# uc-vision/taichi_gaussian_rasterizer

Hardware: AMD Instinct MI355X
Metric: Mpixels/s fwd+bwd @ 2048x2048, 1M Gaussians (higher is better)
Workload: dtype f32

## Files before the change

taichi_gaussian_rasterizer_amd/csrc/frame.cpp:

```cpp

#include <string.h>

#include "gs_common.h"

namespace {

int64_t a256(int64_t bytes) { return gs_align_up(bytes > 0 ? bytes : 1, 256); }

struct Dims {
  int64_t n, P, T;
  int C, F, col0, RS, tiles_x, tiles_y, local_h, D;
  bool want_vis;
};

int frame_dims(const GsFrame* f, Dims* d) {
  GS_REQUIRE(f != nullptr, GS_ERR_INVALID_ARGUMENT, "frame: descriptor is NULL");
  if (int rc = gs_check_cfg(&f->cfg)) return rc;
  GS_REQUIRE(f->n >= 0 && f->n < (int64_t(1) << 31), GS_ERR_INVALID_ARGUMENT, "frame: %lld gaussians", (long long)f->n);
  GS_REQUIRE(f->width > 0 && f->height > 0, GS_ERR_INVALID_ARGUMENT, "frame: image size %dx%d", f->width, f->height);
  GS_REQUIRE(f->sh_degree >= -1 && f->sh_degree <= 3, GS_ERR_UNSUPPORTED, "frame: SH degree %d", f->sh_degree);
  GS_REQUIRE(f->channels >= 1 && f->channels <= (f->sh_degree >= 0 ? GS_MAX_SH_CHANNELS : GS_MAX_FEATURES - 2),
             GS_ERR_UNSUPPORTED, "frame: %d feature channels", f->channels);
  const int ts = f->cfg.tile_size;
  GsShard sh;
  if (int rc = gs_make_shard(f->has_shard ? &f->shard : nullptr, int(gs_div_up(f->height, ts)), &sh)) return rc;
  d->n = f->n;
  d->C = f->channels;
  d->F = f->channels + (f->render_depth ? 2 : 0);
  d->col0 = d->F - d->C;
  d->RS = gs_grad_row_floats(d->F);
  d->D = f->sh_degree >= 0 ? (f->sh_degree + 1) * (f->sh_degree + 1) : 1;
  d->tiles_x = int(gs_div_up(f->width, ts));
  d->tiles_y = sh.local_rows;
  int64_t rows = 0;
  if (!f->has_shard) rows = f->height;
  else
    for (int l = 0; l < sh.local_rows; ++l) {
      const int gy = gs_shard_global_row(sh, l);
      const int64_t y0 = int64_t(gy) * ts, y1 = y0 + ts < f->height ? y0 + ts : f->height;
      rows += y1 - y0;
    }
  d->local_h = int(rows);
  d->T = int64_t(d->tiles_x) * d->tiles_y;
  d->P = rows * f->width;
  d->want_vis = f->cfg.compute_visibility || f->cfg.compute_point_heuristic;
  return GS_OK;
}

template <typename T>
T* at(void* base, int64_t off) { return reinterpret_cast<T*>(static_cast<char*>(base) + off); }

struct StageTimer {
  void* const* events;
  int rc = GS_OK;
  void mark(int stage, int end, void* stream) {
    if (!events || !events[2 * stage + end]) return;
    if (hipEventRecord(static_cast<hipEvent_t>(events[2 * stage + end]), static_cast<hipStream_t>(stream)) != hipSuccess) {
      gs_set_error("frame: hipEventRecord of a stage timer failed");
      rc = GS_ERR_LAUNCH;
    }
  }
};

}

int gs_project_fwd_ex(int64_t n, const float* position, const float* log_scaling, const float* rotation,
                      const float* alpha_logit, const float* T_camera_world, const float* projection, int32_t width,
                      int32_t height, double near_plane, double far_plane, const GsRasterConfig* cfg, float* points,
                      float* depth, float* ndc_depth, int64_t* indexes, int32_t* slot_of, int32_t* num_visible,
                      float* depth_features, int32_t depth_features_stride, float* camera_pos, void* scratch,
                      int64_t scratch_bytes, float* zero_rows, int32_t zero_row_floats, const GsMapBinPlan* bin,
                      void* stream);

extern "C" int gs_frame_layout(const GsFrame* f, GsFrameLayout* out) {
  Dims d;
  if (int rc = frame_dims(f, &d)) return rc;
  GS_REQUIRE(out != nullptr, GS_ERR_INVALID_ARGUMENT, "gs_frame_layout: layout is NULL");
  GS_REQUIRE(f->k_capacity >= 1, GS_ERR_INVALID_ARGUMENT, "gs_frame_layout: k_capacity must be >= 1");
  memset(out, 0, sizeof(*out));
  int64_t p = 0;
  auto take = [&](int64_t bytes) { const int64_t o = p; p += a256(bytes); return o; };
  const int64_t n = d.n > 0 ? d.n : 1;
  out->counts = take(8 * 4);
  out->camera_pos = take(3 * 4);
  out->points = take(n * 7 * 4);
  out->depth = take(n * 4);
  out->features = take(n * d.F * 4);
  out->indexes = take(n * 8);
  out->slot_of = take(n * 4);
  out->tile_ranges = take(d.T * 8);
  out->tile_order = take(d.T * 4);
  out->overlap_to_point = take(f->k_capacity * 4);
  out->image = take(d.P * d.F * 4);
  out->alpha = take(d.P * 4);
  out->visibility = d.want_vis ? take(n * 4) : -1;
  out->out_image = f->render_depth ? take(d.P * d.C * 4) : -1;
  out->img_depth = f->render_depth ? take(d.P * 4) : -1;
  out->img_var = f->render_depth ? take(d.P * 4) : -1;
  out->median = f->render_median_depth ? take(d.P * 4) : -1;
  out->grad_rows = f->prepare_backward ? take(n * d.RS * 4) : -1;
  const bool lists = f->has_shard && f->exchange_world > 0;
  out->touched = lists ? take(n * 4) : -1;
  out->owner_counts = lists ? take(64 * 8) : -1;
  out->workspace_bytes = p;
  p = 0;
  out->s_ndc_depth = take(n * 4);
  out->s_pairs = take(f->k_capacity * 8);
  out->s_median_cover = f->render_median_depth ? take(d.P * 4) : -1;
  const int64_t pb = gs_project_scratch_bytes(d.n), mb = gs_map_scratch_bytes(d.n, d.T > 0 ? d.T : 1);
  out->s_stage = take(a256(mb) + pb);
  out->stage_bytes = a256(mb) + pb;
  out->fwd_scratch_bytes = p;
  p = 0;
  out->b_grad_image = f->render_depth ? take(d.P * d.F * 4) : -1;
  out->b_camera = take(gs_project_bwd_scratch_bytes(d.n));
  out->b_grad_rows = f->prepare_backward ? -1 : take(n * d.RS * 4);
  out->bwd_scratch_bytes = p;
  out->num_features = d.F;
  out->grad_row_floats = d.RS;
  out->tiles_x = d.tiles_x;
  out->tiles_y = d.tiles_y;
  out->local_height = d.local_h;
  return GS_OK;
}

extern "C" int gs_frame_fwd(const GsFrame* f, const float* position, const float* log_scaling, const float* rotation,
                            const float* alpha_logit, const float* feature, const float* T_camera_world,
                            const float* projection, void* workspace, int64_t workspace_bytes, void* scratch,
                            int64_t scratch_bytes, int32_t* counts_host, void* counts_event, void* const* stage_events,
                            const float* background, void* stream) {
  StageTimer tm{stage_events};
  Dims d;
  if (int rc = frame_dims(f, &d)) return rc;
  if (int rc = gs_check_background("gs_frame_fwd", f->cfg.use_alpha_blending, background != nullptr, d.col0, d.F))
    return rc;
  GsFrameLayout L;
  if (int rc = gs_frame_layout(f, &L)) return rc;
  GS_REQUIRE(workspace && workspace_bytes >= L.workspace_bytes, GS_ERR_SCRATCH_TOO_SMALL,
             "gs_frame_fwd: workspace %lld < %lld bytes", (long long)workspace_bytes, (long long)L.workspace_bytes);
  GS_REQUIRE(scratch && scratch_bytes >= L.fwd_scratch_bytes, GS_ERR_SCRATCH_TOO_SMALL,
             "gs_frame_fwd: scratch %lld < %lld bytes", (long long)scratch_bytes, (long long)L.fwd_scratch_bytes);
  GS_REQUIRE(d.n > 0, GS_ERR_INVALID_ARGUMENT, "gs_frame_fwd: no gaussians (run the composed operators)");
  GS_REQUIRE(feature != nullptr, GS_ERR_INVALID_ARGUMENT, "gs_frame_fwd: feature is NULL");
  hipStream_t s = static_cast<hipStream_t>(stream);
  const GsRowShard* shard = f->has_shard ? &f->shard : nullptr;
  const GsRasterConfig* cfg = &f->cfg;
  GsRasterConfig rcfg = f->cfg;
  if (f->render_depth) rcfg.forward_cut = f->depth_forward_cut;
  int32_t* counts = at<int32_t>(workspace, L.counts);
  float* cam_pos = at<float>(workspace, L.camera_pos);
  float* points = at<float>(workspace, L.points);
  float* depth = at<float>(workspace, L.depth);
  float* feats = at<float>(workspace, L.features);
  int64_t* indexes = at<int64_t>(workspace, L.indexes);
  int32_t* slot_of = at<int32_t>(workspace, L.slot_of);
  int32_t* tile_ranges = at<int32_t>(workspace, L.tile_ranges);
  int32_t* tile_order = at<int32_t>(workspace, L.tile_order);
  int32_t* o2p = at<int32_t>(workspace, L.overlap_to_point);
  float* image = at<float>(workspace, L.image);
  float* alpha = at<float>(workspace, L.alpha);
  float* vis = L.visibility >= 0 ? at<float>(workspace, L.visibility) : nullptr;
  float* ndc = at<float>(scratch, L.s_ndc_depth);
  void* stage = at<char>(scratch, L.s_stage);
  const int64_t map_bytes = gs_map_scratch_bytes(d.n, d.T > 0 ? d.T : 1);
  void* proj_stage = at<char>(stage, a256(map_bytes));
  const int64_t proj_bytes = L.stage_bytes - a256(map_bytes);

  const bool lists = shard && f->exchange_world > 0 && d.T > 0;
  GS_REQUIRE(f->exchange_world <= 64 && (f->exchange_world == 0 || (f->exchange_rank >= 0 && f->exchange_rank < f->exchange_world)),
             GS_ERR_INVALID_ARGUMENT, "gs_frame_fwd: exchange rank %d of %d", f->exchange_rank, f->exchange_world);
  if (lists && f->sh_degree >= 0 &&
      hipMemsetD32Async(reinterpret_cast<hipDeviceptr_t>(feats), 0x3F000000, size_t(d.n) * d.F, s) != hipSuccess) {
    gs_set_error("gs_frame_fwd: hipMemsetD32Async failed");
    return GS_ERR_LAUNCH;
  }
  GsMapBinPlan bin;
  bin.width = f->width; bin.height = f->height; bin.cfg = cfg; bin.shard = shard; bin.scratch = stage;
  bin.scratch_bytes = map_bytes;
  tm.mark(GS_FWD_PROJECT, 0, stream);
  if (int rc = gs_project_fwd_ex(d.n, position, log_scaling, rotation, alpha_logit, T_camera_world, projection,
                                 f->width, f->height, f->near_plane, f->far_plane, cfg, points, depth, ndc, indexes,
                                 slot_of, counts, f->render_depth ? feats : nullptr, d.F, cam_pos, proj_stage,
                                 proj_bytes, L.grad_rows >= 0 ? at<float>(workspace, L.grad_rows) : nullptr, d.RS,
                                 d.T > 0 ? &bin : nullptr, stream))
    return rc;
  tm.mark(GS_FWD_PROJECT, 1, stream);
  const int32_t* v_dev = counts;
  float* colours = feats + d.col0;
  int rc;
  tm.mark(GS_FWD_COLOURS, 0, stream);
  if (f->sh_degree >= 0 && lists)
    rc = GS_OK;
  else if (f->sh_degree >= 0 && shard)
    rc = gs_sh_fwd_shard(d.n, v_dev, d.C, f->sh_degree, feature, position, indexes, cam_pos, points, f->height, cfg,
                         shard, colours, d.F, stream);
  else if (f->sh_degree >= 0)
    rc = gs_sh_fwd(d.n, v_dev, d.C, f->sh_degree, feature, position, indexes, cam_pos, colours, d.F, stream);
  else
    rc = gs_feature_gather_fwd(d.n, v_dev, d.C, feature, indexes, colours, d.F, stream);
  tm.mark(GS_FWD_COLOURS, 1, stream);
  if (rc) return rc;
  if (vis && hipMemsetAsync(vis, 0, size_t(d.n) * 4, s) != hipSuccess) {
    gs_set_error("gs_frame_fwd: hipMemsetAsync failed");
    return GS_ERR_LAUNCH;
  }
  if (d.T == 0) {
    if (hipMemsetAsync(counts + 1, 0, 28, s) != hipSuccess) { gs_set_error("gs_frame_fwd: memset failed"); return GS_ERR_LAUNCH; }
    if (L.owner_counts >= 0 && hipMemsetAsync(at<char>(workspace, L.owner_counts), 0, 64 * 8, s) != hipSuccess) {
      gs_set_error("gs_frame_fwd: memset failed");
      return GS_ERR_LAUNCH;
    }
    if (counts_host) {
      if (hipMemcpyAsync(counts_host, counts + 4, 16, hipMemcpyDeviceToHost, s) != hipSuccess ||
          hipMemcpyAsync(counts_host + 4, counts, 4, hipMemcpyDeviceToHost, s) != hipSuccess ||
          hipMemcpyAsync(counts_host + 5, counts + 5, 4, hipMemcpyDeviceToHost, s) != hipSuccess) {
        gs_set_error("gs_frame_fwd: count read-back failed");
        return GS_ERR_LAUNCH;
      }
    }
    if (counts_event && hipEventRecord(static_cast<hipEvent_t>(counts_event), s) != hipSuccess) {
      gs_set_error("gs_frame_fwd: hipEventRecord failed");
      return GS_ERR_LAUNCH;
    }
    return tm.rc;
  }
  tm.mark(GS_FWD_MAP_PREPARE, 0, stream);
  if ((rc = gs_map_prepare_ex(d.n, v_dev, points, f->width, f->height, cfg, f->k_capacity, tile_ranges, counts + 4,
                              counts_host, tile_order, shard, stage, map_bytes, 1, stream)))
    return rc;
  tm.mark(GS_FWD_MAP_PREPARE, 1, stream);
  if (counts_event && hipEventRecord(static_cast<hipEvent_t>(counts_event), s) != hipSuccess) {
    gs_set_error("gs_frame_fwd: hipEventRecord failed");
    return GS_ERR_LAUNCH;
  }
  if (lists) {
    int32_t* touched = at<int32_t>(workspace, L.touched);
    if ((rc = gs_map_touched_list(d.n, v_dev, d.T, stage, map_bytes, touched, counts + 1, indexes, d.n,
                                  f->exchange_world, at<int64_t>(workspace, L.owner_counts), f->exchange_rank,
                                  counts + 2, stream)))
      return rc;
    if (f->sh_degree >= 0) {
      tm.mark(GS_FWD_COLOURS, 0, stream);
      if ((rc = gs_sh_fwd_rows(d.n, touched, counts + 1, d.C, f->sh_degree, feature, position, indexes, cam_pos, colours,
                               d.F, stream)))
        return rc;
      tm.mark(GS_FWD_COLOURS, 1, stream);
    }
  }
  const int32_t tile_hint = f->max_tile_hint > 0 ? -f->max_tile_hint : 0;
  tm.mark(GS_FWD_MAP_FINISH, 0, stream);
  if ((rc = gs_map_finish(d.n, v_dev, f->k_capacity, tile_hint, points, ndc, f->width, f->height, cfg, f->use_depth16,
                          tile_ranges, o2p, nullptr, at<char>(scratch, L.s_pairs), shard, stage, map_bytes,
                          stream)))
    return rc;
  tm.mark(GS_FWD_MAP_FINISH, 1, stream);
  tm.mark(GS_FWD_RASTER, 0, stream);
  if ((rc = gs_raster_fwd(d.n, d.F, points, feats, tile_ranges, o2p, f->k_capacity, f->width, f->height, &rcfg,
                          tile_order, counts + 7, image, alpha, vis, shard, background, d.col0, stream)))
    return rc;
  tm.mark(GS_FWD_RASTER, 1, stream);
  if (f->render_depth &&
      (rc = gs_depth_split_fwd(d.P, d.C, image, alpha, 1e-6f, at<float>(workspace, L.out_image),
                               at<float>(workspace, L.img_depth), at<float>(workspace, L.img_var), stream)))
    return rc;
  if (f->render_median_depth) {
    GsRasterConfig pick = f->cfg;
    pick.use_alpha_blending = 0;
    pick.saturate_threshold = 0.5f;
    pick.compute_visibility = 0;
    pick.compute_point_heuristic = 0;
    if ((rc = gs_raster_fwd(d.n, 1, points, depth, tile_ranges, o2p, f->k_capacity, f->width, f->height, &pick,
                            tile_order, counts + 7, at<float>(workspace, L.median),
                            at<float>(scratch, L.s_median_cover), nullptr, shard, nullptr, 0, stream)))
      return rc;
  }
  return tm.rc;
}

namespace {

int frame_bwd(bool compact, const GsFrame* f, const float* position, const float* log_scaling, const float* rotation,
              const float* alpha_logit, const float* feature, const float* T_camera_world, const float* projection,
              void* workspace, int64_t workspace_bytes, void* scratch, int64_t scratch_bytes, int64_t v, int64_t k,
              const float* grad_image, const float* grad_img_depth, const float* grad_img_var, const float* grad_weight,
              const float* attached_points, const float* attached_depth, float* d_position, float* d_log_scaling,
              float* d_rotation, float* d_alpha_logit, float* d_feature, float* d_T_camera_world, float* d_projection,
              float* d_camera_centre, void* const* stage_events, const GsFrameBwdPart* part, void* stream) {
  StageTimer tm{stage_events};
  Dims d;
  if (int rc = frame_dims(f, &d)) return rc;
  GsFrameLayout L;
  if (int rc = gs_frame_layout(f, &L)) return rc;
  const int first = part ? part->first_stage : GS_BWD_RASTER, end = part ? part->end_stage : GS_BWD_STAGES;
  const int64_t lo = part ? part->row_begin : 0, nr = (part ? part->row_end : d.n) - lo;
  GS_REQUIRE(first >= 0 && first < end && end <= GS_BWD_STAGES, GS_ERR_INVALID_ARGUMENT,
             "gs_frame_bwd: stages [%d, %d)", first, end);
  GS_REQUIRE(lo >= 0 && nr >= 0 && lo + nr <= d.n, GS_ERR_INVALID_ARGUMENT, "gs_frame_bwd: rows [%lld, %lld) of %lld",
             (long long)lo, (long long)(lo + nr), (long long)d.n);
  GS_REQUIRE(!compact || !f->has_shard, GS_ERR_UNSUPPORTED,
             "gs_frame_bwd_rows: a sharded frame has no row-compact gradients (grad_mode \"sharded\" is range-shaped)");
  GS_REQUIRE(!compact || (lo == 0 && nr == d.n), GS_ERR_UNSUPPORTED,
             "gs_frame_bwd_rows: a row sub-range [%lld, %lld) of %lld gaussians", (long long)lo, (long long)(lo + nr),
             (long long)d.n);
  GS_REQUIRE(!f->has_shard || first > GS_BWD_RASTER || end <= GS_BWD_COLOURS, GS_ERR_UNSUPPORTED,
             "gs_frame_bwd: a sharded frame exchanges its partial gradients between the rasterizer and the adjoints; "
             "run [GS_BWD_RASTER, GS_BWD_COLOURS) and the later stages in separate calls");
  GS_REQUIRE(workspace && workspace_bytes >= L.workspace_bytes, GS_ERR_SCRATCH_TOO_SMALL,
             "gs_frame_bwd: workspace %lld < %lld bytes", (long long)workspace_bytes, (long long)L.workspace_bytes);
  GS_REQUIRE(scratch && scratch_bytes >= L.bwd_scratch_bytes, GS_ERR_SCRATCH_TOO_SMALL,
             "gs_frame_bwd: scratch %lld < %lld bytes", (long long)scratch_bytes, (long long)L.bwd_scratch_bytes);
  GS_REQUIRE(v >= 0 && v <= d.n && k >= 0 && k <= f->k_capacity, GS_ERR_INVALID_ARGUMENT,
             "gs_frame_bwd: v = %lld, k = %lld", (long long)v, (long long)k);
  GS_REQUIRE(d_position && d_log_scaling && d_rotation && d_alpha_logit && d_feature, GS_ERR_INVALID_ARGUMENT,
             "gs_frame_bwd: NULL gradient output");
  GS_REQUIRE(!grad_weight || f->cfg.use_alpha_blending, GS_ERR_UNSUPPORTED,
             "gs_frame_bwd: grad_weight needs use_alpha_blending");
  GS_REQUIRE(!grad_weight || grad_image || (f->render_depth && (grad_img_depth || grad_img_var)),
             GS_ERR_INVALID_ARGUMENT, "gs_frame_bwd: grad_weight without a grad_image (pass zeros)");
  hipStream_t s = static_cast<hipStream_t>(stream);
  const GsRasterConfig* cfg = &f->cfg;
  const int32_t* counts = at<int32_t>(workspace, L.counts);
  const float* feats = at<float>(workspace, L.features);
  const int32_t* slot_of = at<int32_t>(workspace, L.slot_of) + lo;
  float* rows = L.grad_rows >= 0 ? at<float>(workspace, L.grad_rows) : at<float>(scratch, L.b_grad_rows);
  const bool own_colours = part && part->colour_grads, own_splats = part && part->splat_grads;
  const float* colours = own_colours ? part->colour_grads : rows + 7 + d.col0;
  float* splats = own_splats ? part->splat_grads : rows;
  const int32_t colour_stride = own_colours ? part->colour_stride : d.RS;
  const int32_t splat_stride = own_splats ? part->splat_stride : d.RS;
  int rc;
  if (first <= GS_BWD_RASTER) {
    if (L.grad_rows < 0 && v > 0 && hipMemsetAsync(rows, 0, size_t(v) * d.RS * 4, s) != hipSuccess) {
      gs_set_error("gs_frame_bwd: hipMemsetAsync failed");
      return GS_ERR_LAUNCH;
    }
    const float* g_img = grad_image;
    if (f->render_depth && v > 0 && d.P > 0 && (grad_image || grad_img_depth || grad_img_var)) {
      float* assembled = at<float>(scratch, L.b_grad_image);
      if ((rc = gs_depth_split_bwd(d.P, d.C, at<float>(workspace, L.img_depth), at<float>(workspace, L.alpha), 1e-6f,
                                   grad_image, grad_img_depth, grad_img_var, assembled, stream)))
        return rc;
      g_img = assembled;
    }
    tm.mark(GS_BWD_RASTER, 0, stream);
    if (g_img && v > 0 && d.P > 0 && k > 0 &&
        (rc = gs_raster_bwd(v, d.F, at<float>(workspace, L.points), feats, at<int32_t>(workspace, L.tile_ranges),
                            at<int32_t>(workspace, L.overlap_to_point), k, f->width, f->height, cfg,
                            at<int32_t>(workspace, L.tile_order), counts + 7, at<float>(workspace, L.image), g_img,
                            grad_weight ? at<float>(workspace, L.alpha) : nullptr, grad_weight, rows,
                            f->has_shard ? &f->shard : nullptr, stream)))
      return rc;
    tm.mark(GS_BWD_RASTER, 1, stream);
  }
  if (first <= GS_BWD_COLOURS && end > GS_BWD_COLOURS) {
    tm.mark(GS_BWD_COLOURS, 0, stream);
    if (compact && f->sh_degree >= 0)
      rc = gs_sh_bwd_rows(d.n, v, d.C, f->sh_degree, feature, position, at<int64_t>(workspace, L.indexes),
                          at<float>(workspace, L.camera_pos), colours, colour_stride, feats + d.col0, d.F, d_feature,
                          nullptr, d_camera_centre, stream);
    else if (compact)
      rc = gs_feature_gather_bwd_rows(v, d.C, colours, colour_stride, d_feature, stream);
    else if (f->sh_degree >= 0)
      rc = gs_sh_bwd(nr, v, d.C, f->sh_degree, feature + lo * d.C * d.D, position + 3 * lo,
                     at<int64_t>(workspace, L.indexes), 1, slot_of, at<float>(workspace, L.camera_pos), colours,
                     colour_stride, feats + d.col0, d.F, d_feature, nullptr, d_camera_centre, stream);
    else
      rc = gs_feature_gather_bwd(nr, d.C, slot_of, colours, colour_stride, d_feature, stream);
    tm.mark(GS_BWD_COLOURS, 1, stream);
    if (rc) return rc;
  }
  if (end > GS_BWD_PROJECT) {
    if ((rc = gs_rows_add(v, splat_stride, splats, attached_points, f->render_depth ? attached_depth : nullptr, 7,
                          stream)))
      return rc;
    const bool camera = d_T_camera_world || d_projection;
    const float* gd = f->render_depth ? splats + 7 : (v > 0 ? attached_depth : nullptr);
    tm.mark(GS_BWD_PROJECT, 0, stream);
    if (compact)
      rc = gs_project_bwd_rows(d.n, v, position, log_scaling, rotation, alpha_logit, T_camera_world, projection, f->width,
                               f->height, cfg, at<int64_t>(workspace, L.indexes), splats, splat_stride, gd,
                               f->render_depth ? splats + 8 : nullptr, f->render_depth ? splat_stride : 1, d_position,
                               d_log_scaling, d_rotation, d_alpha_logit, d_T_camera_world, d_projection,
                               camera ? at<char>(scratch, L.b_camera) : nullptr,
                               camera ? gs_project_bwd_scratch_bytes(d.n) : 0, stream);
    else
      rc = gs_project_bwd(nr, v, position + 3 * lo, log_scaling + 3 * lo, rotation + 4 * lo, alpha_logit + lo,
                          T_camera_world, projection, f->width, f->height, cfg, slot_of, splats, splat_stride, gd,
                          f->render_depth ? splats + 8 : nullptr, f->render_depth ? splat_stride : 1, d_position,
                          d_log_scaling, d_rotation, d_alpha_logit, d_T_camera_world, d_projection,
                          camera ? at<char>(scratch, L.b_camera) : nullptr,
                          camera ? gs_project_bwd_scratch_bytes(nr) : 0, stream);
    tm.mark(GS_BWD_PROJECT, 1, stream);
    if (rc) return rc;
  }
  return tm.rc;
}

}

extern "C" int gs_frame_bwd(const GsFrame* f, const float* position, const float* log_scaling, const float* rotation,
                            const float* alpha_logit, const float* feature, const float* T_camera_world,
                            const float* projection, void* workspace, int64_t workspace_bytes, void* scratch,
                            int64_t scratch_bytes, int64_t v, int64_t k, const float* grad_image,
                            const float* grad_img_depth, const float* grad_img_var, const float* grad_weight,
                            const float* attached_points, const float* attached_depth, float* d_position,
                            float* d_log_scaling, float* d_rotation, float* d_alpha_logit, float* d_feature,
                            float* d_T_camera_world, float* d_projection, float* d_camera_centre,
                            void* const* stage_events, const GsFrameBwdPart* part, void* stream) {
  return frame_bwd(false, f, position, log_scaling, rotation, alpha_logit, feature, T_camera_world, projection, workspace,
                   workspace_bytes, scratch, scratch_bytes, v, k, grad_image, grad_img_depth, grad_img_var, grad_weight,
                   attached_points, attached_depth, d_position, d_log_scaling, d_rotation, d_alpha_logit, d_feature,
                   d_T_camera_world, d_projection, d_camera_centre, stage_events, part, stream);
}

extern "C" int gs_frame_bwd_rows(const GsFrame* f, const float* position, const float* log_scaling, const float* rotation,
                                 const float* alpha_logit, const float* feature, const float* T_camera_world,
                                 const float* projection, void* workspace, int64_t workspace_bytes, void* scratch,
                                 int64_t scratch_bytes, int64_t v, int64_t k, const float* grad_image,
                                 const float* grad_img_depth, const float* grad_img_var, const float* grad_weight,
                                 const float* attached_points, const float* attached_depth, float* d_position,
                                 float* d_log_scaling, float* d_rotation, float* d_alpha_logit, float* d_feature,
                                 float* d_T_camera_world, float* d_projection, float* d_camera_centre,
                                 void* const* stage_events, const GsFrameBwdPart* part, void* stream) {
  return frame_bwd(true, f, position, log_scaling, rotation, alpha_logit, feature, T_camera_world, projection, workspace,
                   workspace_bytes, scratch, scratch_bytes, v, k, grad_image, grad_img_depth, grad_img_var, grad_weight,
                   attached_points, attached_depth, d_position, d_log_scaling, d_rotation, d_alpha_logit, d_feature,
                   d_T_camera_world, d_projection, d_camera_centre, stage_events, part, stream);
}
```

taichi_gaussian_rasterizer_amd/csrc/gs_common.h:

```cpp
#pragma once

#include <hip/hip_runtime.h>
#include <stdint.h>
#include <stdio.h>

#include "../../include/gsplat_hip.h"

#define GS_WAVE 64

void gs_set_error(const char* fmt, ...);

#define GS_REQUIRE(cond, status, ...)  \
  do {                                 \
    if (!(cond)) {                     \
      gs_set_error(__VA_ARGS__);       \
      return (status);                 \
    }                                  \
  } while (0)

#define GS_CHECK_LAUNCH(name)                                                   \
  do {                                                                          \
    hipError_t e_ = hipGetLastError();                                          \
    if (e_ != hipSuccess) {                                                     \
      gs_set_error("%s: launch failed: %s", name, hipGetErrorString(e_));       \
      return GS_ERR_LAUNCH;                                                     \
    }                                                                           \
  } while (0)

static inline int64_t gs_div_up(int64_t a, int64_t b) { return (a + b - 1) / b; }
static inline int64_t gs_align_up(int64_t a, int64_t b) { return gs_div_up(a, b) * b; }

static inline int gs_memset_async(void* ptr, size_t bytes, hipStream_t stream, const char* what) {
  if (hipMemsetAsync(ptr, 0, bytes, stream) == hipSuccess) return GS_OK;
  gs_set_error("%s", what);
  return GS_ERR_LAUNCH;
}

static inline int gs_check_cfg(const GsRasterConfig* cfg) {
  GS_REQUIRE(cfg != nullptr, GS_ERR_INVALID_ARGUMENT, "config is NULL");
  GS_REQUIRE(cfg->tile_size == 8 || cfg->tile_size == 16 || cfg->tile_size == 32, GS_ERR_UNSUPPORTED,
             "tile_size %d not supported (8, 16 or 32)", cfg->tile_size);
  GS_REQUIRE(cfg->alpha_threshold > 0.f, GS_ERR_INVALID_ARGUMENT, "alpha_threshold must be > 0");
  return GS_OK;
}

static inline int gs_check_background(const char* what, int blend, bool has_background, int offset, int num_features) {
  if (!has_background) return GS_OK;
  GS_REQUIRE(blend, GS_ERR_UNSUPPORTED, "%s: a background needs use_alpha_blending (nothing is composited without it)",
             what);
  GS_REQUIRE(offset >= 0 && offset < num_features, GS_ERR_INVALID_ARGUMENT,
             "%s: background_offset %d outside the %d feature channels", what, offset, num_features);
  return GS_OK;
}

static inline int gs_check_raster_call(const char* what, int width, int height, int num_features, int max_features) {
  GS_REQUIRE(width > 0 && height > 0, GS_ERR_INVALID_ARGUMENT, "%s: image size %dx%d", what, width, height);
  GS_REQUIRE(num_features >= 1 && num_features <= max_features, GS_ERR_UNSUPPORTED,
             "%s: feature width %d not in [1,%d]", what, num_features, max_features);
  return GS_OK;
}

static inline int gs_check_raster_fwd_buffers(const char* what, const void* image, const void* alpha,
                                              const void* tile_ranges, int64_t k, const void* points,
                                              const void* features, const void* overlap_to_point, bool vis,
                                              const void* visibility, int64_t v) {
  GS_REQUIRE(image && alpha && tile_ranges, GS_ERR_INVALID_ARGUMENT, "%s: NULL output or ranges", what);
  GS_REQUIRE(k == 0 || (points && features && overlap_to_point), GS_ERR_INVALID_ARGUMENT,
             "%s: NULL input with %lld overlaps", what, (long long)k);
  GS_REQUIRE(!vis || visibility || v == 0, GS_ERR_INVALID_ARGUMENT, "%s: visibility buffer is NULL", what);
  return GS_OK;
}

struct GsShard {
  int begin, end, band, period, phase;
  int local_rows;
};

#ifdef __HIPCC__
#define GS_HD __host__ __device__ __forceinline__
#else
#define GS_HD inline
#endif

GS_HD bool gs_shard_owns(const GsShard& s, int ty) {
  if (ty < s.begin || ty >= s.end) return false;
  return s.period == 1 || (ty / s.band) % s.period == s.phase;
}
GS_HD int gs_shard_local_row(const GsShard& s, int ty) {
  return s.period == 1 ? ty - s.begin : (ty / (s.band * s.period)) * s.band + ty % s.band;
}
GS_HD int gs_shard_global_row(const GsShard& s, int local) {
  return s.period == 1 ? local + s.begin : (local / s.band) * s.band * s.period + s.phase * s.band + local % s.band;
}

GS_HD bool gs_shard_any_row(const GsShard& s, int lo, int hi) {
  lo = lo > s.begin ? lo : s.begin;
  hi = hi < s.end ? hi : s.end;
  if (lo >= hi) return false;
  if (s.period == 1 || hi - lo >= s.band * s.period) return true;
  for (int ty = lo; ty < hi; ++ty)
    if ((ty / s.band) % s.period == s.phase) return true;
  return false;
}

static inline int gs_make_shard(const GsRowShard* shard, int rows, GsShard* out) {
  if (shard == nullptr) {
    out->begin = 0; out->end = rows; out->band = rows > 0 ? rows : 1; out->period = 1; out->phase = 0;
    out->local_rows = rows;
    return GS_OK;
  }
  GS_REQUIRE(shard->row_begin >= 0 && shard->row_begin <= shard->row_end && shard->row_end <= rows,
             GS_ERR_INVALID_ARGUMENT, "shard rows [%d, %d) outside the image's %d tile rows", shard->row_begin,
             shard->row_end, rows);
  out->begin = shard->row_begin; out->end = shard->row_end;
  if (shard->period <= 1) {
    out->band = rows > 0 ? rows : 1; out->period = 1; out->phase = 0;
    out->local_rows = out->end - out->begin;
    return GS_OK;
  }
  GS_REQUIRE(shard->band >= 1 && shard->phase >= 0 && shard->phase < shard->period, GS_ERR_INVALID_ARGUMENT,
             "shard band %d period %d phase %d", shard->band, shard->period, shard->phase);
  GS_REQUIRE(shard->row_begin == 0 && shard->row_end == rows, GS_ERR_INVALID_ARGUMENT,
             "an interleaved shard covers all tile rows (got [%d, %d) of %d)", shard->row_begin, shard->row_end, rows);
  out->band = shard->band; out->period = shard->period; out->phase = shard->phase;
  const int cycle = shard->band * shard->period, full = rows / cycle, rem = rows % cycle;
  int tail = rem - shard->phase * shard->band;
  tail = tail < 0 ? 0 : (tail > shard->band ? shard->band : tail);
  out->local_rows = full * shard->band + tail;
  return GS_OK;
}

int gs_raster_sub_blocks(const GsRasterConfig* cfg, int64_t num_tiles, int backward);

int gs_project_fwd_ex(int64_t n, const float* position, const float* log_scaling, const float* rotation,
                      const float* alpha_logit, const float* T_camera_world, const float* projection, int32_t width,
                      int32_t height, double near_plane, double far_plane, const GsRasterConfig* cfg, float* points,
                      float* depth, float* ndc_depth, int64_t* indexes, int32_t* slot_of, int32_t* num_visible,
                      float* depth_features, int32_t depth_features_stride, float* camera_pos, void* scratch,
                      int64_t scratch_bytes, float* zero_rows, int32_t zero_row_floats, const struct GsMapBinPlan* bin,
                      void* stream);
struct GsMapBinPlan {
  int32_t width, height;
  const GsRasterConfig* cfg;
  const GsRowShard* shard;
  void* scratch;
  int64_t scratch_bytes;
};
struct GsCompactArgs {
  int64_t n;
  const void* st_rows;
  const int* block_offsets;
  const int* block_counts;
  int num_blocks;
  float inv_far, ndc_denom;
  float* points; float* depth; float* ndc; int64_t* indexes; int* slot_of; int* num_visible;
  float* depth_feat; int depth_feat_stride;
  void* zero_rows; int zero_row_v4;
};
int gs_map_compact_bin(const GsMapBinPlan* plan, const GsCompactArgs* c, void* stream);
int gs_map_bin_counters(const GsMapBinPlan* plan, int64_t n, int32_t** words, int32_t* count);
int gs_map_prepare_ex(int64_t v, const int32_t* v_dev, const float* points, int32_t width, int32_t height,
                      const GsRasterConfig* cfg, int64_t k_capacity, int32_t* tile_ranges, int32_t* counts_out,
                      int32_t* counts_host, int32_t* tile_order, const GsRowShard* shard, void* scratch,
                      int64_t scratch_bytes, int binned, void* stream);
int gs_map_sort_tiles(int num_tiles, const int32_t* tile_ranges, uint64_t* pairs, int32_t* overlap_to_point,
                      uint64_t* sorted_keys, int32_t use_depth16, int32_t max_tile_count, hipStream_t stream);
int gs_rows_add(int64_t v, int32_t row_floats, float* rows, const float* add_points, const float* add_depth,
                int32_t depth_col, void* stream);

#ifdef __HIPCC__

__device__ __forceinline__ int gs_xcd_remap(int block, int n) {
  const int chunk = (n + 7) >> 3;
  const int item = (block & 7) * chunk + (block >> 3);
  return ((block >> 3) < chunk && item < n) ? item : -1;
}

template <int CTRL, int ROW_MASK = 0xf, int BANK_MASK = 0xf>
__device__ __forceinline__ float gs_dpp_add(float x) {
  const int moved = __builtin_amdgcn_update_dpp(0, __float_as_int(x), CTRL, ROW_MASK, BANK_MASK, false);
  return x + __int_as_float(moved);
}

__device__ __forceinline__ float gs_wave_sum_to_lane63(float x) {
  x = gs_dpp_add<0x128>(x);
  x = gs_dpp_add<0x124>(x);
  x = gs_dpp_add<0x122>(x);
  x = gs_dpp_add<0x121>(x);
  x = gs_dpp_add<0x142, 0xa>(x);
  x = gs_dpp_add<0x143, 0xc>(x);
  return x;
}

template <int CTRL>
__device__ __forceinline__ float gs_dpp_add_full(float x) {
  return x + __int_as_float(__builtin_amdgcn_mov_dpp(__float_as_int(x), CTRL, 0xf, 0xf, true));
}

__device__ __forceinline__ float gs_wave_reduce16_transposed(float (&v)[16], int lane) {
  float a[8];
#pragma unroll
  for (int i = 0; i < 8; ++i) {
    const auto r = __builtin_amdgcn_permlane32_swap(__float_as_uint(v[i]), __float_as_uint(v[i + 8]), false, false);
    a[i] = __uint_as_float(r[0]) + __uint_as_float(r[1]);
  }
  float b[4];
#pragma unroll
  for (int i = 0; i < 4; ++i) {
    const auto r = __builtin_amdgcn_permlane16_swap(__float_as_uint(a[i]), __float_as_uint(a[i + 4]), false, false);
    b[i] = __uint_as_float(r[0]) + __uint_as_float(r[1]);
  }
  const bool hi8 = (lane & 8) != 0, hi4 = (lane & 4) != 0;
  float c[2];
#pragma unroll
  for (int i = 0; i < 2; ++i) {
    const float t = gs_dpp_add_full<0x128>(b[i]);
    const float u = gs_dpp_add_full<0x128>(b[i + 2]);
    c[i] = hi8 ? u : t;
  }
  const float t = gs_dpp_add_full<0x141>(c[0]);
  const float u = gs_dpp_add_full<0x141>(c[1]);
  float d = hi4 ? u : t;
  d = gs_dpp_add_full<0xB1>(d);
  d = gs_dpp_add_full<0x4E>(d);
  return d;
}

template <int N>
struct GsReduceShape {
  static constexpr int h1 = (N + 1) / 2, h2 = (h1 + 1) / 2, h3 = (h2 + 1) / 2, h4 = (h3 + 1) / 2;
  static_assert(N >= 1 && N <= 16 && h4 == 1, "one register must remain after four halvings");
};

template <int N>
__device__ __forceinline__ int gs_reduce_slot(int lane) {
  typedef GsReduceShape<N> S;
  const int row = lane >> 4, col = lane & 15;
  const int ci = (col >> 2) & 1;
  if (ci >= S::h3) return -1;
  const int bi = ci + ((col >> 3) & 1) * S::h3;
  if (bi >= S::h2) return -1;
  const int ai = bi + (row & 1) * S::h2;
  if (ai >= S::h1) return -1;
  const int vi = ai + (row >> 1) * S::h1;
  return vi < N ? vi : -1;
}

template <int N>
__device__ __forceinline__ float gs_wave_reduce_transposed(float (&v)[N], int lane) {
  typedef GsReduceShape<N> S;
  float a[S::h1];
#pragma unroll
  for (int i = 0; i < S::h1; ++i) {
    const float partner = (i + S::h1 < N) ? v[i + S::h1 < N ? i + S::h1 : 0] : 0.0f;
    const auto r = __builtin_amdgcn_permlane32_swap(__float_as_uint(v[i]), __float_as_uint(partner), false, false);
    a[i] = __uint_as_float(r[0]) + __uint_as_float(r[1]);
  }
  float b[S::h2];
#pragma unroll
  for (int i = 0; i < S::h2; ++i) {
    const float partner = (i + S::h2 < S::h1) ? a[i + S::h2 < S::h1 ? i + S::h2 : 0] : 0.0f;
    const auto r = __builtin_amdgcn_permlane16_swap(__float_as_uint(a[i]), __float_as_uint(partner), false, false);
    b[i] = __uint_as_float(r[0]) + __uint_as_float(r[1]);
  }
  const bool hi8 = (lane & 8) != 0, hi4 = (lane & 4) != 0;
  float c[S::h3];
#pragma unroll
  for (int i = 0; i < S::h3; ++i) {
    const float t = gs_dpp_add_full<0x128>(b[i]);
    if (i + S::h3 < S::h2) {
      const float u = gs_dpp_add_full<0x128>(b[i + S::h3 < S::h2 ? i + S::h3 : 0]);
      c[i] = hi8 ? u : t;
    } else {
      c[i] = t;
    }
  }
  float d = gs_dpp_add_full<0x141>(c[0]);
  if (S::h3 > 1) {
    const float u = gs_dpp_add_full<0x141>(c[S::h3 > 1 ? 1 : 0]);
    d = hi4 ? u : d;
  }
  d = gs_dpp_add_full<0xB1>(d);
  d = gs_dpp_add_full<0x4E>(d);
  return d;
}

template <>
__device__ __forceinline__ int gs_reduce_slot<9>(int lane) {
  return lane == 60 ? 8 : gs_reduce_slot<8>(lane);
}

template <>
__device__ __forceinline__ float gs_wave_reduce_transposed<9>(float (&v)[9], int lane) {
  float w[8];
#pragma unroll
  for (int i = 0; i < 8; ++i) w[i] = v[i];
  float x = v[8];
  x = gs_dpp_add_full<0x128>(x);
  x = gs_dpp_add_full<0x124>(x);
  x = gs_dpp_add_full<0x122>(x);
  x = gs_dpp_add_full<0x121>(x);
  x = gs_dpp_add_full<0x142>(x);
  x = gs_dpp_add_full<0x143>(x);
  const float d = gs_wave_reduce_transposed<8>(w, lane);
  return lane == 60 ? x : d;
}

struct GsCompactSlot {
  int first;
  int slot;
  int total;
};
template <int WAVES>
__device__ __forceinline__ GsCompactSlot gs_stable_compact(bool flag, const int* offset, const int* block_counts,
                                                           int blocks_before) {
  __shared__ int s_cnt[WAVES];
  __shared__ int s_before[WAVES];
  const uint64_t b = __ballot(flag);
  const int wave = threadIdx.x >> 6, lane = threadIdx.x & 63;
  if (lane == 0) s_cnt[wave] = __popcll(b);
  if (!offset) {
    int before = 0;
    for (int j = threadIdx.x; j < blocks_before; j += WAVES * 64) before += block_counts[j];
    for (int off = 32; off > 0; off >>= 1) before += __shfl_xor(before, off);
    if (lane == 0) s_before[wave] = before;
  }
  __syncthreads();
  GsCompactSlot c;
  c.first = 0;
  if (offset) {
    c.first = *offset;
  } else {
#pragma unroll
    for (int w = 0; w < WAVES; ++w) c.first += s_before[w];
  }
  int base = c.first;
  c.total = 0;
#pragma unroll
  for (int w = 0; w < WAVES; ++w) {
    base += w < wave ? s_cnt[w] : 0;
    c.total += s_cnt[w];
  }
  c.slot = base + __popcll(b & ((1ull << lane) - 1ull));
  return c;
}

__device__ __forceinline__ void gs_write_compact_row(const GsCompactArgs& c, int slot, int64_t i, const float4& r0,
                                                     const float4& r1) {
  float* p = c.points + int64_t(slot) * 7;
  p[0] = r0.x; p[1] = r0.y; p[2] = r0.z; p[3] = r0.w; p[4] = r1.x; p[5] = r1.y; p[6] = r1.z;
  c.depth[slot] = r1.w;
  if (c.depth_feat) {
    c.depth_feat[int64_t(slot) * c.depth_feat_stride] = r1.w;
    c.depth_feat[int64_t(slot) * c.depth_feat_stride + 1] = r1.w * r1.w;
  }
  const float inv_d = __fdiv_rn(1.0f, r1.w);
  c.ndc[slot] = 1.0f - __fdiv_rn(inv_d - c.inv_far, c.ndc_denom);
  c.indexes[slot] = i;
}

__device__ __forceinline__ float gs_exp2_fast(float x) { return __builtin_amdgcn_exp2f(x); }
__device__ __forceinline__ float gs_rcp_fast(float x) { return __builtin_amdgcn_rcpf(x); }

template <int NB>
__device__ __forceinline__ int gs_sub_block_mask(float Ax, float Ay, float Bx, float By, float r2, float relx,
                                                 float rely) {
  const float sxx = Ax * Ax + Bx * Bx, sxy = Ax * Ay + Bx * By, syy = Ay * Ay + By * By;
  const float rxy = -sxy * gs_rcp_fast(syy), ryx = -sxy * gs_rcp_fast(sxx);
  const float lim = r2 * 1.002f + 1e-3f;
  int mask = 0;
#pragma unroll
  for (int b = 0; b < NB; ++b) {
    const float xa = relx + float((b & 1) * 8), ya = rely + float((b >> 1) * 8);
    const float xb = xa + 7.0f, yb = ya + 7.0f;
    const float xn = __builtin_amdgcn_fmed3f(0.0f, xa, xb), yn = __builtin_amdgcn_fmed3f(0.0f, ya, yb);
    const float ys = __builtin_amdgcn_fmed3f(rxy * xn, ya, yb);
    const float xs = __builtin_amdgcn_fmed3f(ryx * yn, xa, xb);
    const float t1x = Ax * xn + Ay * ys, t1y = Bx * xn + By * ys;
    const float t2x = Ax * xs + Ay * yn, t2y = Bx * xs + By * yn;
    const float q1 = t1x * t1x + t1y * t1y, q2 = t2x * t2x + t2y * t2y;
    if (fminf(q1, q2) <= lim) mask |= 1 << b;
  }
  return mask;
}

template <int NB>
__device__ __forceinline__ int gs_sub_block_mask_antialias(float ax, float ay, float sx, float sy, float alpha,
                                                           float inv_thr, float d0x, float d0y, float relx, float rely) {
  const float base = alpha * 6.28318530717958648f * sx * sy * inv_thr;
  const float Lx = __logf(base * d0y), Ly = __logf(base * d0x);
  if (!(Lx > 0.0f && Ly > 0.0f)) return 0;
  const float zx = fminf(Lx * 0.625f, cbrtf(Lx * 14.2857142857f)), zy = fminf(Ly * 0.625f, cbrtf(Ly * 14.2857142857f));
  const float X = (0.5f + sx * zx) * 1.001f + 0.01f, Y = (0.5f + sy * zy) * 1.001f + 0.01f;
  const float h = 3.5f * (fabsf(ax) + fabsf(ay));
  const float ex = 3.5f + X * fabsf(ax) + Y * fabsf(ay), ey = 3.5f + X * fabsf(ay) + Y * fabsf(ax);
  int mask = 0;
#pragma unroll
  for (int b = 0; b < NB; ++b) {
    const float cx = relx + float((b & 1) * 8) + 3.5f, cy = rely + float((b >> 1) * 8) + 3.5f;
    if (fabsf(cx * ax + cy * ay) <= X + h && fabsf(cy * ax - cx * ay) <= Y + h && fabsf(cx) <= ex && fabsf(cy) <= ey)
      mask |= 1 << b;
  }
  return mask;
}

#endif
```

taichi_gaussian_rasterizer_amd/csrc/mapper.hip:

```cpp

#include "map_query.h"

namespace {

__global__ __launch_bounds__(1024) void map_scan_kernel(int num_tiles, const int* tile_hist, int2* tile_ranges,
                                                        int* cursors, int* counts_out, int64_t k_capacity,
                                                        int* tile_order, const int* v_dev, int* counts_host,
                                                        const int* touched_dev) {
  __shared__ int s_wave[16];
  __shared__ int s_bin[1024];
  const int t = threadIdx.x;
  if (blockIdx.x == 0) {
    constexpr int PER = 16;
    int carry = 0, mx = 0;
    for (int base0 = 0; base0 < num_tiles; base0 += 1024 * PER) {
      const int i0 = base0 + t * PER;
      int c[PER];
      const bool whole = i0 + PER <= num_tiles;
      if (whole) {
        const int4* src = reinterpret_cast<const int4*>(tile_hist + i0);
#pragma unroll
        for (int q = 0; q < PER / 4; ++q) {
          const int4 v4 = src[q];
          c[4 * q] = v4.x; c[4 * q + 1] = v4.y; c[4 * q + 2] = v4.z; c[4 * q + 3] = v4.w;
        }
      } else {
#pragma unroll
        for (int j = 0; j < PER; ++j) c[j] = i0 + j < num_tiles ? tile_hist[i0 + j] : 0;
      }
      int sum = 0;
#pragma unroll
      for (int j = 0; j < PER; ++j) { sum += c[j]; mx = max(mx, c[j]); }
      int total;
      int run = carry + block_exclusive_scan(sum, s_wave, total);
      carry += total;
      int2 rg[PER];
      int cur[PER];
#pragma unroll
      for (int j = 0; j < PER; ++j) {
        const bool fits = k_capacity <= 0 || int64_t(run) + c[j] <= k_capacity;
        rg[j] = (c[j] > 0 && fits) ? make_int2(run, run + c[j]) : make_int2(0, 0);
        cur[j] = fits ? run : -(1 << 30);
        run += c[j];
      }
      if (whole) {
        int4* dr = reinterpret_cast<int4*>(tile_ranges + i0);
        int4* dc = reinterpret_cast<int4*>(cursors + i0);
#pragma unroll
        for (int q = 0; q < PER / 2; ++q) dr[q] = make_int4(rg[2 * q].x, rg[2 * q].y, rg[2 * q + 1].x, rg[2 * q + 1].y);
#pragma unroll
        for (int q = 0; q < PER / 4; ++q) dc[q] = make_int4(cur[4 * q], cur[4 * q + 1], cur[4 * q + 2], cur[4 * q + 3]);
      } else {
#pragma unroll
        for (int j = 0; j < PER; ++j)
          if (i0 + j < num_tiles) { tile_ranges[i0 + j] = rg[j]; cursors[i0 + j] = cur[j]; }
      }
    }
    for (int off = 32; off > 0; off >>= 1) mx = max(mx, __shfl_xor(mx, off));
    if ((t & 63) == 0) s_wave[t >> 6] = mx;
    __syncthreads();
    if (t == 0) {
      int m = 0;
      for (int w = 0; w < 16; ++w) m = max(m, s_wave[w]);
      const int over = (k_capacity > 0 && int64_t(carry) > k_capacity) ? 1 : 0;
      counts_out[0] = carry;
      counts_out[1] = m;
      counts_out[2] = over;
      if (!tile_order) counts_out[3] = 0;
      if (counts_host) {
        counts_host[0] = carry;
        counts_host[1] = m;
        counts_host[2] = over;
        if (!tile_order) counts_host[3] = 0;
        counts_host[4] = v_dev ? *v_dev : 0;
        counts_host[5] = touched_dev ? *touched_dev : 0;
      }
    }
    return;
  }
  constexpr int PER = 16;
  s_bin[t] = 0;
  __syncthreads();
  int sum = 0;
  int c0[PER];
  for (int base0 = 0; base0 < num_tiles; base0 += 1024 * PER) {
    const int i0 = base0 + t * PER;
    int c[PER];
    if (i0 + PER <= num_tiles) {
      const int4* src = reinterpret_cast<const int4*>(tile_hist + i0);
#pragma unroll
      for (int q = 0; q < PER / 4; ++q) {
        const int4 v4 = src[q];
        c[4 * q] = v4.x; c[4 * q + 1] = v4.y; c[4 * q + 2] = v4.z; c[4 * q + 3] = v4.w;
      }
    } else {
#pragma unroll
      for (int j = 0; j < PER; ++j) c[j] = i0 + j < num_tiles ? tile_hist[i0 + j] : -1;
    }
#pragma unroll
    for (int j = 0; j < PER; ++j) {
      if (base0 == 0) c0[j] = c[j];
      if (c[j] >= 0) {
        sum += c[j];
        atomicAdd(&s_bin[min(c[j], 1023)], 1);
      }
    }
  }
  int unused, k_total;
  block_exclusive_scan(sum, s_wave, k_total);
  const int start = block_exclusive_scan(s_bin[1023 - t], s_wave, unused);
  s_bin[1023 - t] = start;
  {
    const int thr_bin = min(max(k_total / 1792, 96), 1022);
    if (1023 - t == thr_bin) {
      const int heavy = min(start, num_tiles / 4);
      counts_out[3] = heavy;
      if (counts_host) counts_host[3] = heavy;
    }
  }
  __syncthreads();
  for (int base0 = 0; base0 < num_tiles; base0 += 1024 * PER) {
    const int i0 = base0 + t * PER;
#pragma unroll
    for (int j = 0; j < PER; ++j) {
      const int c = base0 == 0 ? c0[j] : (i0 + j < num_tiles ? tile_hist[i0 + j] : -1);
      if (c >= 0 && i0 + j < num_tiles) tile_order[atomicAdd(&s_bin[min(c, 1023)], 1)] = i0 + j;
    }
  }
}

constexpr int RG_MIN = 8;
constexpr int RB = 4;
constexpr int MAX_REGIONS = 1024;
constexpr int WIDE_SPAN = 64;
#ifndef GS_MAP_CHUNK
#define GS_MAP_CHUNK 512
#endif
constexpr int CHUNK = GS_MAP_CHUNK;

struct RegionGrid {
  int tiles_x, tiles_y, regions_x, num_regions;
  int rg;
  int win;
  int row0;
};

struct QueryCache {
  unsigned long long accept;
  unsigned int x;
  unsigned int y;
};
constexpr unsigned QC_WIDE = 0x80000000u;
__device__ __forceinline__ int qc_min_tx(const QueryCache& q) { return int(q.x & 0xfffffu); }
__device__ __forceinline__ int qc_min_ty(const QueryCache& q) { return int(q.y & 0xfffffu); }
__device__ __forceinline__ int qc_span_x(const QueryCache& q) { return int((q.x >> 20) & 0x7fu); }

struct Window {
  int x0, y0, win;
  __device__ __forceinline__ Window(const RegionGrid& rg, int region)
      : x0((region % rg.regions_x) * rg.rg - RB), y0((region / rg.regions_x) * rg.rg - RB + rg.row0), win(rg.win) {}
  __device__ __forceinline__ bool slot(int gx, int gy, int& e) const {
    const int lx = gx - x0, ly = gy - y0;
    e = ly * win + lx;
    return unsigned(lx) < unsigned(win) && unsigned(ly) < unsigned(win);
  }
  __device__ __forceinline__ void tile_of(int e, int& gx, int& gy) const { gx = x0 + e % win; gy = y0 + e / win; }
};

template <typename F>
__device__ __forceinline__ void for_each_accepted(unsigned long long accept, int span_x, F f) {
  for (unsigned long long todo = accept; todo != 0ull; todo &= todo - 1ull) {
    const int bit = __ffsll(todo) - 1;
    const int ty = bit / span_x, tx = bit - ty * span_x;
    f(tx, ty);
  }
}

template <typename F>
__device__ __forceinline__ void for_each_wide_tile(const MapArgs& a, int i, uint64_t wide_lanes, F f) {
  for (uint64_t todo = wide_lanes; todo != 0ull; todo &= todo - 1ull) {
    const int gi = __shfl(i, __ffsll(static_cast<unsigned long long>(todo)) - 1);
    const GridQuery q = grid_query(a.points + 7 * int64_t(gi), a.Wp, a.Hp, a.tile_size, a.thr);
    auto g = f(gi);
    const int total = q.span_x * q.span_y;
    for (int k = int(threadIdx.x & 63); k < total; k += 64) {
      const int ty = k / q.span_x, tx = k - ty * q.span_x;
      if (gs_shard_owns(a.sh, ty + q.min_ty) && test_tile(q, tx, ty, a.tile_size)) g(tx + q.min_tx, ty + q.min_ty);
    }
  }
}

__device__ __forceinline__ bool enters_order(const float* g, const MapArgs& a) {
  if (a.sh.period == 1 && a.sh.begin == 0 && a.sh.end * a.tile_size >= a.Hp) return true;
  const GridQuery q = grid_query(g, a.Wp, a.Hp, a.tile_size, a.thr);
  return q.span_x > 0 && gs_shard_any_row(a.sh, q.min_ty, q.min_ty + q.span_y);
}

__device__ __forceinline__ int region_of_gaussian(const float* g, const MapArgs& a, const RegionGrid& rg) {
  const float ts = float(a.tile_size);
  int tx = int(floorf(g[0] / ts)), ty = int(floorf(g[1] / ts));
  tx = min(max(tx, 0), rg.tiles_x - 1);
  ty = min(max(ty - rg.row0, 0), rg.tiles_y - 1);
  return (ty / rg.rg) * rg.regions_x + (tx / rg.rg);
}

constexpr int BIN = 1024;
__device__ __forceinline__ void publish_region_hist(const int* s_hist, const RegionGrid& rg, int num_wg, int blk,
                                                    int* part, int* region_count) {
  for (int r = threadIdx.x; r < rg.num_regions; r += BIN) {
    const int h = s_hist[r];
    if (region_count == nullptr) part[int64_t(r) * num_wg + blk] = h;
    else if (h > 0) part[int64_t(r) * num_wg + blk] = atomicAdd(region_count + r, h);
  }
}

__device__ __forceinline__ void bin_row(bool active, const float* g, const MapArgs& a, const RegionGrid& rg,
                                        int* region_of_row, int* s_hist, int first, int rows, int num_wg,
                                        int* touched_blocks, int* block_start) {
  bool binned = false;
  if (active) {
    const bool any = enters_order(g, a);
    const int r = any ? region_of_gaussian(g, a, rg) : -1;
    *region_of_row = r;
    if (r >= 0) atomicAdd(&s_hist[r], 1);
    binned = r >= 0;
  }
  const int touched = __syncthreads_count(binned);
  if (threadIdx.x == 0) {
    touched_blocks[blockIdx.x] = touched;
    block_start[blockIdx.x] = first;
    if (int(blockIdx.x) == num_wg - 1) block_start[num_wg] = first + rows;
  }
}

__global__ __launch_bounds__(BIN) void region_count_kernel(MapArgs a, RegionGrid rg, int num_wg, int* region_of,
                                                           int* part, int* touched_blocks, int* block_start,
                                                           int* region_count) {
  __shared__ int s_hist[MAX_REGIONS];
  for (int r = threadIdx.x; r < rg.num_regions; r += BIN) s_hist[r] = 0;
  __syncthreads();
  const int64_t i = int64_t(blockIdx.x) * BIN + threadIdx.x;
  const int64_t live = live_count(a);
  const int first = int(min(int64_t(blockIdx.x) * BIN, live));
  bin_row(i < live, a.points + 7 * i, a, rg, region_of + i, s_hist, first, int(live) - first, num_wg, touched_blocks,
          block_start);
  publish_region_hist(s_hist, rg, num_wg, blockIdx.x, part, region_count);
}

__global__ __launch_bounds__(1024) void region_part_scan_kernel(int num_wg, int* part, int* region_count) {
  __shared__ int s_wave[16];
  const int total = block_scan_row_in_place(part + int64_t(blockIdx.x) * num_wg, num_wg, s_wave);
  if (threadIdx.x == 0) region_count[blockIdx.x] = total;
}

__device__ __forceinline__ int scan_region_starts(int num_regions, const int* region_count, int* s_wave, bool publish,
                                                  int* region_start, int* chunk_start) {
  const int r = threadIdx.x;
  const int c = r < num_regions ? region_count[r] : 0;
  int total_c;
  const int start = block_exclusive_scan(c, s_wave, total_c);
  if (publish) {
    int total_ch;
    const int chunk = block_exclusive_scan((c + CHUNK - 1) / CHUNK, s_wave, total_ch);
    if (r < num_regions) {
      region_start[r] = start;
      chunk_start[r] = chunk;
    }
    if (r == 0) {
      region_start[num_regions] = total_c;
      chunk_start[num_regions] = total_ch;
    }
  }
  return start;
}

__global__ __launch_bounds__(1024) void region_scan_kernel(int num_regions, const int* region_count, int* region_start,
                                                           int* chunk_start) {
  __shared__ int s_wave[16];
  scan_region_starts(num_regions, region_count, s_wave, true, region_start, chunk_start);
}

__global__ __launch_bounds__(BIN) void region_scatter_kernel(RegionGrid rg, int num_wg, const int* region_of,
                                                             const int* part, const int* region_count,
                                                             int* region_start, int* chunk_start,
                                                             const int* block_start, int* order, int* tile_hist,
                                                             int num_tiles, int scanned) {
  __shared__ int s_cnt[MAX_REGIONS];
  __shared__ int s_start[MAX_REGIONS];
  __shared__ int s_wave[16];
  for (int i = blockIdx.x * BIN + threadIdx.x; i < num_tiles; i += gridDim.x * BIN) tile_hist[i] = 0;
  const int t = threadIdx.x;
  s_cnt[t] = 0;
  if (scanned) {
    s_start[t] = t < rg.num_regions ? region_start[t] : 0;
  } else {
    s_start[t] = scan_region_starts(rg.num_regions, region_count, s_wave, blockIdx.x == 0, region_start, chunk_start);
  }
  __syncthreads();
  const int first = block_start[blockIdx.x];
  const int i = first + t;
  if (i < block_start[blockIdx.x + 1]) {
    const int r = region_of[i];
    if (r >= 0) {
      const int local = atomicAdd(&s_cnt[r], 1);
      order[s_start[r] + part[int64_t(r) * num_wg + blockIdx.x] + local] = i;
    }
  }
}

__global__ __launch_bounds__(BIN) void compact_bin_kernel(GsCompactArgs c, MapArgs a, RegionGrid rg, int num_wg,
                                                          int* region_of, int* part, int* touched_blocks,
                                                          int* block_start, int* region_count) {
  __shared__ int s_hist[MAX_REGIONS];
  for (int r = threadIdx.x; r < rg.num_regions; r += BIN) s_hist[r] = 0;
  const int64_t i = int64_t(blockIdx.x) * BIN + threadIdx.x;
  const float4* st_rows = static_cast<const float4*>(c.st_rows);
  float4 r0 = make_float4(0, 0, 0, 0), r1 = r0;
  bool vis = false;
  if (i < c.n) {
    r0 = st_rows[2 * i];
    r1 = st_rows[2 * i + 1];
    vis = r1.w != 0.0f;
  }
  const int first_small = int(blockIdx.x) * (BIN / 256);
  const GsCompactSlot k = gs_stable_compact<BIN / 64>(vis, c.block_offsets ? c.block_offsets + first_small : nullptr,
                                                      c.block_counts, first_small);
  const int first = k.first, mine_total = k.total;
  if (i < c.n) {
    if (vis) gs_write_compact_row(c, k.slot, i, r0, r1);
    c.slot_of[i] = vis ? k.slot : -1;
  }
  const float g[7] = {r0.x, r0.y, r0.z, r0.w, r1.x, r1.y, r1.z};
  bin_row(vis, g, a, rg, region_of + k.slot, s_hist, first, mine_total, num_wg, touched_blocks, block_start);
  if (threadIdx.x == 0 && int(blockIdx.x) == num_wg - 1) *c.num_visible = first + mine_total;
  const int my_hist = int(threadIdx.x) < rg.num_regions ? s_hist[threadIdx.x] : 0;
  int my_offset = my_hist;
  if (region_count != nullptr && my_hist > 0) my_offset = atomicAdd(region_count + threadIdx.x, my_hist);
  if (c.zero_rows) {
    float4* dst = static_cast<float4*>(c.zero_rows) + int64_t(first) * c.zero_row_v4;
    for (int e = threadIdx.x; e < mine_total * c.zero_row_v4; e += BIN) dst[e] = make_float4(0, 0, 0, 0);
  }
  if (int(threadIdx.x) < rg.num_regions && (region_count == nullptr || my_hist > 0))
    part[int64_t(threadIdx.x) * num_wg + blockIdx.x] = my_offset;
}

__device__ __forceinline__ bool locate_chunk(int block, const RegionGrid& rg, const int* region_start,
                                             const int* chunk_start, int& region, int& first, int& count) {
  __shared__ int s_loc[3];
  if (threadIdx.x == 0) {
    int r = -1;
    if (block < chunk_start[rg.num_regions]) {
      int lo = 0, hi = rg.num_regions;
      while (hi - lo > 1) {
        const int mid = (lo + hi) >> 1;
        if (chunk_start[mid] <= block) lo = mid; else hi = mid;
      }
      r = lo;
      const int c = block - chunk_start[r];
      s_loc[1] = region_start[r] + c * CHUNK;
      s_loc[2] = min(CHUNK, region_start[r + 1] - s_loc[1]);
    }
    s_loc[0] = r;
  }
  __syncthreads();
  region = s_loc[0];
  first = s_loc[1];
  count = s_loc[2];
  return region >= 0;
}

__global__ __launch_bounds__(CHUNK) void count_binned_kernel(MapArgs a, RegionGrid rg, const int* order,
                                                           const int* region_start, const int* chunk_start,
                                                           int* tile_hist, QueryCache* qcache) {
  extern __shared__ int s_win[];
  const int WIN_TILES = rg.win * rg.win;
  int region, first, count;
  if (!locate_chunk(blockIdx.x, rg, region_start, chunk_start, region, first, count)) return;
  for (int e = threadIdx.x; e < WIN_TILES; e += CHUNK) s_win[e] = 0;
  __syncthreads();
  const Window w(rg, region);
  auto add_tile = [&](int gx, int gy) {
    int e;
    if (w.slot(gx, gy, e)) atomicAdd(&s_win[e], 1);
    else atomicAdd(tile_hist + local_tile(a, gx, gy), 1);
  };
  int i = 0;
  bool wide = false;
  if (int(threadIdx.x) < count) {
    i = order[first + threadIdx.x];
    const GridQuery q = grid_query(a.points + 7 * int64_t(i), a.Wp, a.Hp, a.tile_size, a.thr);
    wide = q.span_x * q.span_y > WIDE_SPAN;
    QueryCache qc;
    qc.accept = 0ull;
    qc.x = unsigned(q.min_tx) | (wide ? 0u : unsigned(q.span_x) << 20);
    qc.y = unsigned(q.min_ty) | (wide ? QC_WIDE : unsigned(q.span_y) << 20);
    if (!wide) {
      int bit = 0;
      for (int ty = 0; ty < q.span_y; ++ty)
        for (int tx = 0; tx < q.span_x; ++tx, ++bit)
          if (gs_shard_owns(a.sh, ty + q.min_ty) && test_tile(q, tx, ty, a.tile_size)) {
            qc.accept |= 1ull << bit;
            add_tile(tx + q.min_tx, ty + q.min_ty);
          }
    }
    *reinterpret_cast<uint4*>(qcache + first + threadIdx.x) = *reinterpret_cast<const uint4*>(&qc);
  }
  for_each_wide_tile(a, i, __ballot(wide), [&](int) { return add_tile; });
  __syncthreads();
  for (int e = threadIdx.x; e < WIN_TILES; e += CHUNK) {
    const int c = s_win[e];
    if (c > 0) {
      int gx, gy;
      w.tile_of(e, gx, gy);
      atomicAdd(tile_hist + local_tile(a, gx, gy), c);
    }
  }
}

__global__ __launch_bounds__(CHUNK) void emit_binned_kernel(MapArgs a, RegionGrid rg, const int* order,
                                                          const int* region_start, const int* chunk_start,
                                                          int* cursors, uint64_t* pairs, const QueryCache* qcache) {
  extern __shared__ int s_dyn[];
  const int WIN_TILES = rg.win * rg.win;
  int* s_cnt = s_dyn;
  int* s_base = s_dyn + WIN_TILES;
  int region, first, count;
  if (!locate_chunk(blockIdx.x, rg, region_start, chunk_start, region, first, count)) return;
  for (int e = threadIdx.x; e < WIN_TILES; e += CHUNK) s_cnt[e] = 0;
  __syncthreads();
  const Window w(rg, region);
  const bool active = int(threadIdx.x) < count;
  unsigned long long accept = 0ull;
  int min_tx = 0, min_ty = 0, span_x = 1;
  bool wide = false;
  int i = 0;
  auto count_tile = [&](int gx, int gy) {
    int e;
    if (w.slot(gx, gy, e)) atomicAdd(&s_cnt[e], 1);
  };
  if (active) {
    i = order[first + threadIdx.x];
    const uint4 raw = *reinterpret_cast<const uint4*>(qcache + first + threadIdx.x);
    const QueryCache qc = *reinterpret_cast<const QueryCache*>(&raw);
    wide = (qc.y & QC_WIDE) != 0u;
    if (!wide) {
      accept = qc.accept;
      min_tx = qc_min_tx(qc); min_ty = qc_min_ty(qc); span_x = qc_span_x(qc);
      for_each_accepted(accept, span_x, [&](int tx, int ty) { count_tile(tx + min_tx, ty + min_ty); });
    }
  }
  const uint64_t wide_lanes = __ballot(wide);
  for_each_wide_tile(a, i, wide_lanes, [&](int) { return count_tile; });
  __syncthreads();
  for (int e = threadIdx.x; e < WIN_TILES; e += CHUNK) {
    const int c = s_cnt[e];
    if (c > 0) {
      int gx, gy;
      w.tile_of(e, gx, gy);
      const int base = atomicAdd(cursors + local_tile(a, gx, gy), c);
      s_base[e] = base < 0 ? -1 : base;
    }
    s_cnt[e] = 0;
  }
  __syncthreads();
  auto place = [&](int gx, int gy, uint64_t pair) {
    int e;
    int slot;
    if (w.slot(gx, gy, e)) {
      if (s_base[e] < 0) return;
      slot = s_base[e] + atomicAdd(&s_cnt[e], 1);
    } else {
      slot = atomicAdd(cursors + local_tile(a, gx, gy), 1);
      if (slot < 0) return;
    }
    pairs[slot] = pair;
  };
  auto pair_of = [&](int gi) {
    return (uint64_t(depth_key(a.depth[gi], a.depth16 != 0)) << 32) | uint64_t(uint32_t(gi));
  };
  if (active && !wide) {
    const uint64_t pair = pair_of(i);
    for_each_accepted(accept, span_x, [&](int tx, int ty) { place(tx + min_tx, ty + min_ty, pair); });
  }
  for_each_wide_tile(a, i, wide_lanes, [&](int gi) {
    const uint64_t pair = pair_of(gi);
    return [&place, pair](int gx, int gy) { place(gx, gy, pair); };
  });
}

struct MapScratch {
  int* hist; int* cursors; int* region_of; int* order; int* region_count; int* region_start; int* part;
  int* chunk_start;
  QueryCache* qcache;
  int* touched_blocks;
  int* block_start;
  char* end;
};
int64_t part_entries(int64_t v, int64_t num_tiles) {
  const int64_t regions = num_tiles < MAX_REGIONS ? (num_tiles < 1 ? 1 : num_tiles) : MAX_REGIONS;
  return regions * gs_div_up(v > 0 ? v : 1, BIN);
}
MapScratch carve(void* scratch, int64_t v, int64_t num_tiles) {
  char* p = static_cast<char*>(scratch);
  MapScratch m;
  auto take = [&](int64_t bytes) { int* r = reinterpret_cast<int*>(p); p += gs_align_up(bytes, 256); return r; };
  m.hist = take(num_tiles * 4);
  m.cursors = take(num_tiles * 4);
  m.region_of = take(v * 4);
  m.order = take(v * 4);
  m.region_count = take((MAX_REGIONS + 1) * 4);
  m.region_start = take((MAX_REGIONS + 1) * 4);
  m.chunk_start = take((MAX_REGIONS + 1) * 4);
  m.part = take(part_entries(v, num_tiles) * 4);
  m.qcache = reinterpret_cast<QueryCache*>(take(v * int64_t(sizeof(QueryCache))));
  m.touched_blocks = take((gs_div_up(v > 0 ? v : 1, BIN) + 1) * 4);
  m.block_start = take((gs_div_up(v > 0 ? v : 1, BIN) + 1) * 4);
  m.end = p;
  return m;
}
RegionGrid make_grid(const MapArgs& a) {
  RegionGrid rg;
  rg.tiles_x = a.tiles_wide;
  rg.row0 = a.sh.period == 1 ? a.sh.begin : 0;
  rg.tiles_y = a.sh.period == 1 ? a.sh.end - a.sh.begin : a.Hp / a.tile_size;
  rg.rg = RG_MIN;
  while (gs_div_up(rg.tiles_x, rg.rg) * gs_div_up(rg.tiles_y, rg.rg) > MAX_REGIONS) rg.rg *= 2;
  rg.win = rg.rg + 2 * RB;
  rg.regions_x = int(gs_div_up(rg.tiles_x, rg.rg));
  rg.num_regions = rg.regions_x * int(gs_div_up(rg.tiles_y, rg.rg));
  return rg;
}

bool bin_with_atomics(int64_t num_wg, const RegionGrid& rg) { return num_wg * rg.num_regions <= (int64_t(1) << 16); }

__global__ __launch_bounds__(1024) void touched_write_kernel(const int* block_start, const int* region_of,
                                                             const int* block_counts, int* touched, int* count_out) {
  const int i = block_start[blockIdx.x] + int(threadIdx.x);
  const bool flag = i < block_start[blockIdx.x + 1] && region_of[i] >= 0;
  const GsCompactSlot k = gs_stable_compact<16>(flag, nullptr, block_counts, int(blockIdx.x));
  if (flag) touched[k.slot] = i;
  if (count_out && blockIdx.x == gridDim.x - 1 && threadIdx.x == 0) *count_out = k.first + k.total;
}

__global__ void owner_cuts_kernel(const int* block_counts, int num_blocks, const int* touched, const int64_t* indexes,
                                  int64_t chunk, int world, int64_t* owner_counts, const int* v_dev, int64_t v,
                                  int owner, int* owned_rows) {
  __shared__ int64_t s_cut[65];
  __shared__ int s_part[128];
  const int t = threadIdx.x;
  int part = 0;
  for (int j = t; j < num_blocks; j += 128) part += block_counts[j];
  s_part[t] = part;
  __syncthreads();
  int m = 0;
  for (int j = 0; j < 128; ++j) m += s_part[j];
  if (t <= world) {
    const int64_t bound = int64_t(t) * chunk;
    int lo = 0, hi = m;
    while (lo < hi) {
      const int mid = (lo + hi) >> 1;
      if (indexes[touched[mid]] < bound) lo = mid + 1; else hi = mid;
    }
    s_cut[t] = t == world ? m : lo;
  }
  __syncthreads();
  if (t < world) owner_counts[t] = s_cut[t + 1] - s_cut[t];
  if (owned_rows && t >= 126) {
    const int64_t bound = int64_t(owner + (t - 126)) * chunk;
    int64_t lo = 0, hi = v_dev ? (int64_t(*v_dev) < v ? int64_t(*v_dev) : v) : v;
    while (lo < hi) {
      const int64_t mid = (lo + hi) >> 1;
      if (indexes[mid] < bound) lo = mid + 1; else hi = mid;
    }
    owned_rows[t - 126] = int(lo);
  }
}
}

extern "C" int64_t gs_map_scratch_bytes(int64_t v, int64_t num_tiles) {
  return carve(nullptr, v, num_tiles).end - static_cast<char*>(nullptr);
}

extern "C" int64_t gs_map_touched_offset(int64_t v, int64_t num_tiles) {
  const MapScratch m = carve(nullptr, v, num_tiles);
  return reinterpret_cast<char*>(m.order) - static_cast<char*>(nullptr);
}

extern "C" int gs_map_touched_list(int64_t v, const int32_t* v_dev, int64_t num_tiles, const void* scratch,
                                   int64_t scratch_bytes, int32_t* touched_out, int32_t* count_out,
                                   const int64_t* indexes, int64_t n, int32_t world, int64_t* owner_counts,
                                   int32_t owner, int32_t* owned_rows, void* stream) {
  GS_REQUIRE(v >= 0 && v < (int64_t(1) << 31) && num_tiles >= 1, GS_ERR_INVALID_ARGUMENT, "gs_map_touched_list: sizes");
  hipStream_t s = static_cast<hipStream_t>(stream);
  if (owner_counts) {
    GS_REQUIRE(world >= 1 && world <= 64 && indexes && n >= 0, GS_ERR_INVALID_ARGUMENT,
               "gs_map_touched_list: %d owners (1 .. 64) need the index list", world);
    if (int rc = gs_memset_async(owner_counts, size_t(world) * 8, s, "gs_map_touched_list: hipMemsetAsync failed"))
      return rc;
  }
  if (count_out && v == 0)
    if (int rc = gs_memset_async(count_out, 4, s, "gs_map_touched_list: hipMemsetAsync failed")) return rc;
  if (v == 0) return GS_OK;
  const int nb = int(gs_div_up(v, 1024));
  GS_REQUIRE(scratch && scratch_bytes >= gs_map_scratch_bytes(v, num_tiles), GS_ERR_SCRATCH_TOO_SMALL,
             "gs_map_touched_list: scratch is not the one gs_map_prepare filled");
  GS_REQUIRE(touched_out, GS_ERR_INVALID_ARGUMENT, "gs_map_touched_list: touched_out is NULL");
  const MapScratch m = carve(const_cast<void*>(scratch), v, num_tiles);
  const int* block_counts = m.touched_blocks;
  hipLaunchKernelGGL(touched_write_kernel, dim3(nb), dim3(1024), 0, s, m.block_start, m.region_of, block_counts,
                     touched_out, count_out);
  if (owner_counts) {
    GS_REQUIRE(!owned_rows || (owner >= 0 && owner < world), GS_ERR_INVALID_ARGUMENT,
               "gs_map_touched_list: owned_rows needs the owner's rank");
    hipLaunchKernelGGL(owner_cuts_kernel, dim3(1), dim3(128), 0, s, block_counts, nb, touched_out, indexes,
                       gs_div_up(n > 0 ? n : 1, world), world, owner_counts, v_dev, v, owner, owned_rows);
  }
  GS_CHECK_LAUNCH("gs_map_touched_list");
  return GS_OK;
}

int gs_map_bin_counters(const GsMapBinPlan* plan, int64_t n, int32_t** words, int32_t* count) {
  MapArgs a;
  if (int rc = fill_args(a, n, nullptr, nullptr, plan->width, plan->height, plan->cfg, 0, plan->shard)) return rc;
  GS_REQUIRE(a.sh.local_rows > 0 && plan->scratch, GS_ERR_INVALID_ARGUMENT, "gs_map_bin_counters: nothing to bin");
  const MapScratch m = carve(plan->scratch, n, int64_t(a.tiles_wide) * a.sh.local_rows);
  const bool atomics = bin_with_atomics(gs_div_up(n > 0 ? n : 1, BIN), make_grid(a));
  *words = atomics ? m.region_count : nullptr;
  *count = atomics ? MAX_REGIONS + 1 : 0;
  return GS_OK;
}

int gs_map_compact_bin(const GsMapBinPlan* plan, const GsCompactArgs* c, void* stream) {
  MapArgs a;
  if (int rc = fill_args(a, c->n, c->points, nullptr, plan->width, plan->height, plan->cfg, 0, plan->shard)) return rc;
  GS_REQUIRE(a.sh.local_rows > 0 && c->n > 0, GS_ERR_INVALID_ARGUMENT, "gs_map_compact_bin: nothing to bin");
  const int num_tiles = a.tiles_wide * a.sh.local_rows;
  GS_REQUIRE(plan->scratch && plan->scratch_bytes >= gs_map_scratch_bytes(c->n, num_tiles), GS_ERR_SCRATCH_TOO_SMALL,
             "gs_map_compact_bin: mapper scratch %lld < %lld bytes", (long long)plan->scratch_bytes,
             (long long)gs_map_scratch_bytes(c->n, num_tiles));
  const RegionGrid rg = make_grid(a);
  GS_REQUIRE(rg.num_regions <= MAX_REGIONS, GS_ERR_UNSUPPORTED, "gs_map_compact_bin: %d regions", rg.num_regions);
  const MapScratch m = carve(plan->scratch, c->n, num_tiles);
  const unsigned vb = unsigned(gs_div_up(c->n, BIN));
  hipLaunchKernelGGL(compact_bin_kernel, dim3(vb), dim3(BIN), 0, static_cast<hipStream_t>(stream), *c, a, rg, int(vb),
                     m.region_of, m.part, m.touched_blocks, m.block_start,
                     bin_with_atomics(vb, rg) ? m.region_count : nullptr);
  GS_CHECK_LAUNCH("gs_map_compact_bin");
  return GS_OK;
}

extern "C" int gs_map_prepare(int64_t v, const int32_t* v_dev, const float* points, int32_t width, int32_t height,
                              const GsRasterConfig* cfg, int64_t k_capacity, int32_t* tile_ranges,
                              int32_t* counts_out, int32_t* counts_host, int32_t* tile_order,
                              const GsRowShard* shard, void* scratch, int64_t scratch_bytes, void* stream) {
  return gs_map_prepare_ex(v, v_dev, points, width, height, cfg, k_capacity, tile_ranges, counts_out, counts_host,
                           tile_order, shard, scratch, scratch_bytes, 0, stream);
}

int gs_map_prepare_ex(int64_t v, const int32_t* v_dev, const float* points, int32_t width, int32_t height,
                      const GsRasterConfig* cfg, int64_t k_capacity, int32_t* tile_ranges, int32_t* counts_out,
                      int32_t* counts_host, int32_t* tile_order, const GsRowShard* shard, void* scratch,
                      int64_t scratch_bytes, int binned, void* stream) {
  MapArgs a;
  if (int rc = fill_args(a, v, points, nullptr, width, height, cfg, 0, shard)) return rc;
  a.v_dev = v_dev;
  GS_REQUIRE(a.sh.local_rows > 0, GS_ERR_INVALID_ARGUMENT, "gs_map_prepare: the shard owns no tile row");
  const int num_tiles = a.tiles_wide * a.sh.local_rows;
  GS_REQUIRE(tile_ranges && counts_out && scratch, GS_ERR_INVALID_ARGUMENT, "gs_map_prepare: NULL buffer");
  GS_REQUIRE(scratch_bytes >= gs_map_scratch_bytes(v, num_tiles), GS_ERR_SCRATCH_TOO_SMALL,
             "gs_map_prepare: scratch %lld < %lld bytes", (long long)scratch_bytes,
             (long long)gs_map_scratch_bytes(v, num_tiles));
  GS_REQUIRE(num_tiles <= (1 << 20), GS_ERR_UNSUPPORTED, "gs_map_prepare: %d tiles (limit 2^20)", num_tiles);
  hipStream_t s = static_cast<hipStream_t>(stream);
  const MapScratch m = carve(scratch, v, num_tiles);
  int* hist = m.hist;
  int* cursors = m.cursors;
  const RegionGrid rg = make_grid(a);
  GS_REQUIRE(rg.num_regions <= MAX_REGIONS && rg.win * rg.win * 8 <= 65536, GS_ERR_UNSUPPORTED,
             "gs_map_prepare: tile grid %dx%d needs %d regions of edge %d", rg.tiles_x, rg.tiles_y, rg.num_regions,
             rg.rg);
  if (v == 0)
    if (int rc = gs_memset_async(hist, size_t(num_tiles) * 4, s, "gs_map_prepare: hipMemsetAsync failed")) return rc;
  if (v > 0) {
    GS_REQUIRE(points, GS_ERR_INVALID_ARGUMENT, "gs_map_prepare: points is NULL");
    const unsigned vb = unsigned(gs_div_up(v, BIN));
    const bool atomics = bin_with_atomics(vb, rg);
    if (!binned) {
      if (atomics)
        if (int rc = gs_memset_async(m.region_count, size_t(MAX_REGIONS + 1) * 4, s,
                                     "gs_map_prepare: hipMemsetAsync failed"))
          return rc;
      hipLaunchKernelGGL(region_count_kernel, dim3(vb), dim3(BIN), 0, s, a, rg, int(vb), m.region_of, m.part,
                         m.touched_blocks, m.block_start, atomics ? m.region_count : nullptr);
    }
    if (!atomics) {
      hipLaunchKernelGGL(region_part_scan_kernel, dim3(rg.num_regions), dim3(1024), 0, s, int(vb), m.part,
                         m.region_count);
      hipLaunchKernelGGL(region_scan_kernel, dim3(1), dim3(1024), 0, s, rg.num_regions, m.region_count,
                         m.region_start, m.chunk_start);
    }
    hipLaunchKernelGGL(region_scatter_kernel, dim3(vb), dim3(BIN), 0, s, rg, int(vb), m.region_of, m.part,
                       m.region_count, m.region_start, m.chunk_start, m.block_start, m.order, hist, num_tiles,
                       atomics ? 0 : 1);
    hipLaunchKernelGGL(count_binned_kernel, dim3(unsigned(gs_div_up(v, CHUNK)) + unsigned(rg.num_regions)), dim3(CHUNK),
                       size_t(rg.win) * rg.win * 4, s, a, rg, m.order,
                       m.region_start, m.chunk_start, hist, m.qcache);
    GS_CHECK_LAUNCH("gs_map_prepare/count");
  }
  hipLaunchKernelGGL(map_scan_kernel, dim3(tile_order ? 2 : 1), dim3(1024), 0, s, num_tiles, hist,
                     reinterpret_cast<int2*>(tile_ranges), cursors, counts_out, k_capacity, tile_order, v_dev,
                     counts_host, v > 0 ? m.region_start + rg.num_regions : nullptr);
  GS_CHECK_LAUNCH("gs_map_prepare/scan");
  return GS_OK;
}

extern "C" int gs_map_finish(int64_t v, const int32_t* v_dev, int64_t k, int32_t max_tile_count, const float* points,
                             const float* depth, int32_t width, int32_t height, const GsRasterConfig* cfg,
                             int32_t use_depth16, const int32_t* tile_ranges, int32_t* overlap_to_point,
                             uint64_t* sorted_keys, void* pair_scratch, const GsRowShard* shard, void* scratch,
                             int64_t scratch_bytes, void* stream) {
  MapArgs a;
  if (int rc = fill_args(a, v, points, depth, width, height, cfg, use_depth16, shard)) return rc;
  a.v_dev = v_dev;
  if (k == 0 || v == 0) return GS_OK;
  const int num_tiles = a.tiles_wide * a.sh.local_rows;
  GS_REQUIRE(points && depth && tile_ranges && overlap_to_point && pair_scratch && scratch, GS_ERR_INVALID_ARGUMENT,
             "gs_map_finish: NULL buffer");
  GS_REQUIRE(scratch_bytes >= gs_map_scratch_bytes(v, num_tiles), GS_ERR_SCRATCH_TOO_SMALL,
             "gs_map_finish: scratch too small");
  hipStream_t s = static_cast<hipStream_t>(stream);
  const MapScratch m = carve(scratch, v, num_tiles);
  int* cursors = m.cursors;
  const RegionGrid rg = make_grid(a);
  uint64_t* pairs = static_cast<uint64_t*>(pair_scratch);
  hipLaunchKernelGGL(emit_binned_kernel, dim3(unsigned(gs_div_up(v, CHUNK)) + unsigned(rg.num_regions)), dim3(CHUNK),
                     size_t(rg.win) * rg.win * 8, s,
                     a, rg, m.order, m.region_start, m.chunk_start, cursors, pairs, m.qcache);
  GS_CHECK_LAUNCH("gs_map_finish/emit");
  return gs_map_sort_tiles(num_tiles, tile_ranges, pairs, overlap_to_point, sorted_keys, use_depth16, max_tile_count, s);
}
```

Baseline: 4001.

## Bin gaussians into region-contiguous records with run table instead of index order

Replaces the count/part-scan/scatter binning pipeline with a single bin pass that writes each workgroup's gaussians, grouped by region, as packed 32-byte records plus depth keys. A new runs kernel scans per-region run lengths and emits chunk descriptors, so downstream count/emit kernels read contiguous records rather than gathering through an order index. The emit step can then use the precomputed NDC depth key instead of reading depth separately. This cuts kernel launches and random gathers, at the cost of extra scratch memory for duplicated rows and a per-chunk binary search over runs.

```diff
diff --git a/taichi_gaussian_rasterizer_amd/csrc/frame.cpp b/taichi_gaussian_rasterizer_amd/csrc/frame.cpp
--- a/taichi_gaussian_rasterizer_amd/csrc/frame.cpp
+++ b/taichi_gaussian_rasterizer_amd/csrc/frame.cpp
@@ -249,9 +249,9 @@
   }
   const int32_t tile_hint = f->max_tile_hint > 0 ? -f->max_tile_hint : 0;
   tm.mark(GS_FWD_MAP_FINISH, 0, stream);
-  if ((rc = gs_map_finish(d.n, v_dev, f->k_capacity, tile_hint, points, ndc, f->width, f->height, cfg, f->use_depth16,
-                          tile_ranges, o2p, nullptr, at<char>(scratch, L.s_pairs), shard, stage, map_bytes,
-                          stream)))
+  if ((rc = gs_map_finish_ex(d.n, v_dev, f->k_capacity, tile_hint, points, ndc, f->width, f->height, cfg,
+                             f->use_depth16, tile_ranges, o2p, nullptr, at<char>(scratch, L.s_pairs), shard, stage,
+                             map_bytes, 1, stream)))
     return rc;
   tm.mark(GS_FWD_MAP_FINISH, 1, stream);
   tm.mark(GS_FWD_RASTER, 0, stream);
diff --git a/taichi_gaussian_rasterizer_amd/csrc/gs_common.h b/taichi_gaussian_rasterizer_amd/csrc/gs_common.h
--- a/taichi_gaussian_rasterizer_amd/csrc/gs_common.h
+++ b/taichi_gaussian_rasterizer_amd/csrc/gs_common.h
@@ -163,6 +163,10 @@
                       const GsRasterConfig* cfg, int64_t k_capacity, int32_t* tile_ranges, int32_t* counts_out,
                       int32_t* counts_host, int32_t* tile_order, const GsRowShard* shard, void* scratch,
                       int64_t scratch_bytes, int binned, void* stream);
+int gs_map_finish_ex(int64_t v, const int32_t* v_dev, int64_t k, int32_t max_tile_count, const float* points,
+                     const float* depth, int32_t width, int32_t height, const GsRasterConfig* cfg, int32_t use_depth16,
+                     const int32_t* tile_ranges, int32_t* overlap_to_point, uint64_t* sorted_keys, void* pair_scratch,
+                     const GsRowShard* shard, void* scratch, int64_t scratch_bytes, int binned, void* stream);
 int gs_map_sort_tiles(int num_tiles, const int32_t* tile_ranges, uint64_t* pairs, int32_t* overlap_to_point,
                       uint64_t* sorted_keys, int32_t use_depth16, int32_t max_tile_count, hipStream_t stream);
 int gs_rows_add(int64_t v, int32_t row_floats, float* rows, const float* add_points, const float* add_depth,
@@ -345,6 +349,11 @@
   return c;
 }
 
+__device__ __forceinline__ float gs_ndc_depth(const GsCompactArgs& c, float depth) {
+  const float inv_d = __fdiv_rn(1.0f, depth);
+  return 1.0f - __fdiv_rn(inv_d - c.inv_far, c.ndc_denom);
+}
+
 __device__ __forceinline__ void gs_write_compact_row(const GsCompactArgs& c, int slot, int64_t i, const float4& r0,
                                                      const float4& r1) {
   float* p = c.points + int64_t(slot) * 7;
@@ -354,8 +363,7 @@
     c.depth_feat[int64_t(slot) * c.depth_feat_stride] = r1.w;
     c.depth_feat[int64_t(slot) * c.depth_feat_stride + 1] = r1.w * r1.w;
   }
-  const float inv_d = __fdiv_rn(1.0f, r1.w);
-  c.ndc[slot] = 1.0f - __fdiv_rn(inv_d - c.inv_far, c.ndc_denom);
+  c.ndc[slot] = gs_ndc_depth(c, r1.w);
   c.indexes[slot] = i;
 }
 
diff --git a/taichi_gaussian_rasterizer_amd/csrc/mapper.hip b/taichi_gaussian_rasterizer_amd/csrc/mapper.hip
--- a/taichi_gaussian_rasterizer_amd/csrc/mapper.hip
+++ b/taichi_gaussian_rasterizer_amd/csrc/mapper.hip
@@ -179,9 +179,10 @@
 template <typename F>
 __device__ __forceinline__ void for_each_wide_tile(const MapArgs& a, int i, uint64_t wide_lanes, F f) {
   for (uint64_t todo = wide_lanes; todo != 0ull; todo &= todo - 1ull) {
-    const int gi = __shfl(i, __ffsll(static_cast<unsigned long long>(todo)) - 1);
+    const int src = __ffsll(static_cast<unsigned long long>(todo)) - 1;
+    const int gi = __shfl(i, src);
     const GridQuery q = grid_query(a.points + 7 * int64_t(gi), a.Wp, a.Hp, a.tile_size, a.thr);
-    auto g = f(gi);
+    auto g = f(src);
     const int total = q.span_x * q.span_y;
     for (int k = int(threadIdx.x & 63); k < total; k += 64) {
       const int ty = k / q.span_x, tx = k - ty * q.span_x;
@@ -205,114 +206,139 @@
 }
 
 constexpr int BIN = 1024;
-__device__ __forceinline__ void publish_region_hist(const int* s_hist, const RegionGrid& rg, int num_wg, int blk,
-                                                    int* part, int* region_count) {
-  for (int r = threadIdx.x; r < rg.num_regions; r += BIN) {
-    const int h = s_hist[r];
-    if (region_count == nullptr) part[int64_t(r) * num_wg + blk] = h;
-    else if (h > 0) part[int64_t(r) * num_wg + blk] = atomicAdd(region_count + r, h);
-  }
-}
-
-__device__ __forceinline__ void bin_row(bool active, const float* g, const MapArgs& a, const RegionGrid& rg,
-                                        int* region_of_row, int* s_hist, int first, int rows, int num_wg,
-                                        int* touched_blocks, int* block_start) {
-  bool binned = false;
+static_assert(BIN == MAX_REGIONS, "one thread per region in the binning workgroups");
+
+struct BinRecord {
+  float g[7];
+  int row;
+};
+struct BinKey {
+  int row;
+  float depth;
+};
+static_assert(sizeof(BinRecord) == 32 && sizeof(BinKey) == 8, "records are moved as uint4 / uint2");
+struct Run {
+  int pos;
+  int addr;
+};
+struct Chunk {
+  int region, wg0, pos0, count;
+};
+constexpr int NUM_COUNTERS = 2;
+
+struct BinOut {
+  BinRecord* binned;
+  BinKey* keys;
+  Run* runs;
+  int* entered;
+  int* touched_blocks;
+  int* block_start;
+};
+
+__device__ __forceinline__ void bin_rows(bool active, const float* g, int row, float depth, const MapArgs& a,
+                                         const RegionGrid& rg, int first, int rows, int num_wg, const BinOut& o) {
+  __shared__ int s_hist[MAX_REGIONS];
+  __shared__ int s_start[MAX_REGIONS];
+  __shared__ int s_wave[16];
+  __shared__ uint4 s_rec[2 * BIN];
+  __shared__ uint2 s_key[BIN];
+  const int t = threadIdx.x;
+  s_hist[t] = 0;
+  __syncthreads();
+  int r = -1, rank = 0;
   if (active) {
-    const bool any = enters_order(g, a);
-    const int r = any ? region_of_gaussian(g, a, rg) : -1;
-    *region_of_row = r;
-    if (r >= 0) atomicAdd(&s_hist[r], 1);
-    binned = r >= 0;
-  }
-  const int touched = __syncthreads_count(binned);
-  if (threadIdx.x == 0) {
-    touched_blocks[blockIdx.x] = touched;
-    block_start[blockIdx.x] = first;
-    if (int(blockIdx.x) == num_wg - 1) block_start[num_wg] = first + rows;
-  }
-}
-
-__global__ __launch_bounds__(BIN) void region_count_kernel(MapArgs a, RegionGrid rg, int num_wg, int* region_of,
-                                                           int* part, int* touched_blocks, int* block_start,
-                                                           int* region_count) {
-  __shared__ int s_hist[MAX_REGIONS];
-  for (int r = threadIdx.x; r < rg.num_regions; r += BIN) s_hist[r] = 0;
-  __syncthreads();
+    if (enters_order(g, a)) {
+      r = region_of_gaussian(g, a, rg);
+      rank = atomicAdd(&s_hist[r], 1);
+    }
+    if (o.entered) o.entered[row] = r;
+  }
+  __syncthreads();
+  const int h = s_hist[t];
+  int touched;
+  const int start = block_exclusive_scan(h, s_wave, touched);
+  s_start[t] = start;
+  __syncthreads();
+  if (r >= 0) {
+    const int p = s_start[r] + rank;
+    s_rec[2 * p] = make_uint4(__float_as_uint(g[0]), __float_as_uint(g[1]), __float_as_uint(g[2]), __float_as_uint(g[3]));
+    s_rec[2 * p + 1] = make_uint4(__float_as_uint(g[4]), __float_as_uint(g[5]), __float_as_uint(g[6]), unsigned(row));
+    s_key[p] = make_uint2(unsigned(row), __float_as_uint(depth));
+  }
+  if (t == 0) {
+    o.touched_blocks[blockIdx.x] = touched;
+    o.block_start[blockIdx.x] = first;
+    if (int(blockIdx.x) == num_wg - 1) o.block_start[num_wg] = first + rows;
+  }
+  if (t < rg.num_regions) {
+    Run run;
+    run.pos = h;
+    run.addr = first + start;
+    *reinterpret_cast<int2*>(o.runs + int64_t(t) * num_wg + blockIdx.x) = make_int2(run.pos, run.addr);
+  }
+  __syncthreads();
+  uint4* dst = reinterpret_cast<uint4*>(o.binned + first);
+  for (int e = t; e < 2 * touched; e += BIN) dst[e] = s_rec[e];
+  uint2* dk = reinterpret_cast<uint2*>(o.keys + first);
+  for (int e = t; e < touched; e += BIN) dk[e] = s_key[e];
+}
+
+__global__ __launch_bounds__(BIN) void region_bin_kernel(MapArgs a, RegionGrid rg, int num_wg, BinOut o) {
   const int64_t i = int64_t(blockIdx.x) * BIN + threadIdx.x;
   const int64_t live = live_count(a);
   const int first = int(min(int64_t(blockIdx.x) * BIN, live));
-  bin_row(i < live, a.points + 7 * i, a, rg, region_of + i, s_hist, first, int(live) - first, num_wg, touched_blocks,
-          block_start);
-  publish_region_hist(s_hist, rg, num_wg, blockIdx.x, part, region_count);
-}
-
-__global__ __launch_bounds__(1024) void region_part_scan_kernel(int num_wg, int* part, int* region_count) {
+  float g[7] = {0, 0, 0, 0, 0, 0, 0};
+  if (i < live)
+    for (int j = 0; j < 7; ++j) g[j] = a.points[7 * i + j];
+  bin_rows(i < live, g, int(i), 0.0f, a, rg, first, int(min(int64_t(BIN), live - first)), num_wg, o);
+}
+
+__global__ __launch_bounds__(1024) void region_runs_kernel(int num_wg, Run* runs, int* counters, Chunk* chunks,
+                                                           int* tile_hist, int num_tiles) {
   __shared__ int s_wave[16];
-  const int total = block_scan_row_in_place(part + int64_t(blockIdx.x) * num_wg, num_wg, s_wave);
-  if (threadIdx.x == 0) region_count[blockIdx.x] = total;
-}
-
-__device__ __forceinline__ int scan_region_starts(int num_regions, const int* region_count, int* s_wave, bool publish,
-                                                  int* region_start, int* chunk_start) {
-  const int r = threadIdx.x;
-  const int c = r < num_regions ? region_count[r] : 0;
-  int total_c;
-  const int start = block_exclusive_scan(c, s_wave, total_c);
-  if (publish) {
-    int total_ch;
-    const int chunk = block_exclusive_scan((c + CHUNK - 1) / CHUNK, s_wave, total_ch);
-    if (r < num_regions) {
-      region_start[r] = start;
-      chunk_start[r] = chunk;
-    }
-    if (r == 0) {
-      region_start[num_regions] = total_c;
-      chunk_start[num_regions] = total_ch;
-    }
-  }
-  return start;
-}
-
-__global__ __launch_bounds__(1024) void region_scan_kernel(int num_regions, const int* region_count, int* region_start,
-                                                           int* chunk_start) {
-  __shared__ int s_wave[16];
-  scan_region_starts(num_regions, region_count, s_wave, true, region_start, chunk_start);
-}
-
-__global__ __launch_bounds__(BIN) void region_scatter_kernel(RegionGrid rg, int num_wg, const int* region_of,
-                                                             const int* part, const int* region_count,
-                                                             int* region_start, int* chunk_start,
-                                                             const int* block_start, int* order, int* tile_hist,
-                                                             int num_tiles, int scanned) {
-  __shared__ int s_cnt[MAX_REGIONS];
-  __shared__ int s_start[MAX_REGIONS];
-  __shared__ int s_wave[16];
-  for (int i = blockIdx.x * BIN + threadIdx.x; i < num_tiles; i += gridDim.x * BIN) tile_hist[i] = 0;
+  __shared__ int s_base;
   const int t = threadIdx.x;
-  s_cnt[t] = 0;
-  if (scanned) {
-    s_start[t] = t < rg.num_regions ? region_start[t] : 0;
-  } else {
-    s_start[t] = scan_region_starts(rg.num_regions, region_count, s_wave, blockIdx.x == 0, region_start, chunk_start);
-  }
-  __syncthreads();
-  const int first = block_start[blockIdx.x];
-  const int i = first + t;
-  if (i < block_start[blockIdx.x + 1]) {
-    const int r = region_of[i];
-    if (r >= 0) {
-      const int local = atomicAdd(&s_cnt[r], 1);
-      order[s_start[r] + part[int64_t(r) * num_wg + blockIdx.x] + local] = i;
-    }
+  for (int i = blockIdx.x * 1024 + t; i < num_tiles; i += gridDim.x * 1024) tile_hist[i] = 0;
+  Run* row = runs + int64_t(blockIdx.x) * num_wg;
+  const int len0 = t < num_wg ? row[t].pos : 0;
+  int rest = 0;
+  for (int b = t + 1024; b < num_wg; b += 1024) rest += row[b].pos;
+  int sum0;
+  const int s0 = block_exclusive_scan(len0, s_wave, sum0);
+  int total = sum0;
+  if (num_wg > 1024) {
+    int sum_rest;
+    block_exclusive_scan(rest, s_wave, sum_rest);
+    total += sum_rest;
+  }
+  if (t == 0) {
+    s_base = atomicAdd(counters, (total + CHUNK - 1) / CHUNK);
+    atomicAdd(counters + 1, total);
+  }
+  __syncthreads();
+  Chunk* mine_chunks = chunks + s_base;
+  auto place_run = [&](int b, int s, int len) {
+    if (b < num_wg) row[b].pos = s;
+    for (int c = (s + CHUNK - 1) / CHUNK; c * CHUNK < s + len; ++c) {
+      Chunk ch;
+      ch.region = blockIdx.x; ch.wg0 = b; ch.pos0 = c * CHUNK; ch.count = min(CHUNK, total - c * CHUNK);
+      *reinterpret_cast<int4*>(mine_chunks + c) = make_int4(ch.region, ch.wg0, ch.pos0, ch.count);
+    }
+  };
+  place_run(t, s0, len0);
+  int carry = sum0;
+  for (int base = 1024; base < num_wg; base += 1024) {
+    const int b = base + t;
+    const int len = b < num_wg ? row[b].pos : 0;
+    int sum;
+    const int s = carry + block_exclusive_scan(len, s_wave, sum);
+    carry += sum;
+    place_run(b, s, len);
   }
 }
 
 __global__ __launch_bounds__(BIN) void compact_bin_kernel(GsCompactArgs c, MapArgs a, RegionGrid rg, int num_wg,
-                                                          int* region_of, int* part, int* touched_blocks,
-                                                          int* block_start, int* region_count) {
-  __shared__ int s_hist[MAX_REGIONS];
-  for (int r = threadIdx.x; r < rg.num_regions; r += BIN) s_hist[r] = 0;
+                                                          BinOut o) {
   const int64_t i = int64_t(blockIdx.x) * BIN + threadIdx.x;
   const float4* st_rows = static_cast<const float4*>(c.st_rows);
   float4 r0 = make_float4(0, 0, 0, 0), r1 = r0;
@@ -330,52 +356,69 @@
     if (vis) gs_write_compact_row(c, k.slot, i, r0, r1);
     c.slot_of[i] = vis ? k.slot : -1;
   }
+  if (threadIdx.x == 0 && int(blockIdx.x) == num_wg - 1) *c.num_visible = first + mine_total;
   const float g[7] = {r0.x, r0.y, r0.z, r0.w, r1.x, r1.y, r1.z};
-  bin_row(vis, g, a, rg, region_of + k.slot, s_hist, first, mine_total, num_wg, touched_blocks, block_start);
-  if (threadIdx.x == 0 && int(blockIdx.x) == num_wg - 1) *c.num_visible = first + mine_total;
-  const int my_hist = int(threadIdx.x) < rg.num_regions ? s_hist[threadIdx.x] : 0;
-  int my_offset = my_hist;
-  if (region_count != nullptr && my_hist > 0) my_offset = atomicAdd(region_count + threadIdx.x, my_hist);
+  bin_rows(vis, g, k.slot, vis ? gs_ndc_depth(c, r1.w) : 0.0f, a, rg, first, mine_total, num_wg, o);
   if (c.zero_rows) {
     float4* dst = static_cast<float4*>(c.zero_rows) + int64_t(first) * c.zero_row_v4;
     for (int e = threadIdx.x; e < mine_total * c.zero_row_v4; e += BIN) dst[e] = make_float4(0, 0, 0, 0);
   }
-  if (int(threadIdx.x) < rg.num_regions && (region_count == nullptr || my_hist > 0))
-    part[int64_t(threadIdx.x) * num_wg + blockIdx.x] = my_offset;
-}
-
-__device__ __forceinline__ bool locate_chunk(int block, const RegionGrid& rg, const int* region_start,
-                                             const int* chunk_start, int& region, int& first, int& count) {
-  __shared__ int s_loc[3];
-  if (threadIdx.x == 0) {
-    int r = -1;
-    if (block < chunk_start[rg.num_regions]) {
-      int lo = 0, hi = rg.num_regions;
-      while (hi - lo > 1) {
-        const int mid = (lo + hi) >> 1;
-        if (chunk_start[mid] <= block) lo = mid; else hi = mid;
-      }
-      r = lo;
-      const int c = block - chunk_start[r];
-      s_loc[1] = region_start[r] + c * CHUNK;
-      s_loc[2] = min(CHUNK, region_start[r + 1] - s_loc[1]);
-    }
-    s_loc[0] = r;
-  }
-  __syncthreads();
-  region = s_loc[0];
-  first = s_loc[1];
-  count = s_loc[2];
-  return region >= 0;
-}
-
-__global__ __launch_bounds__(CHUNK) void count_binned_kernel(MapArgs a, RegionGrid rg, const int* order,
-                                                           const int* region_start, const int* chunk_start,
-                                                           int* tile_hist, QueryCache* qcache) {
+}
+
+struct RunTable {
+  const BinRecord* binned;
+  const BinKey* keys;
+  const Run* runs;
+  const Chunk* chunks;
+  const int* counters;
+  int num_wg;
+};
+
+__device__ __forceinline__ int locate_record(int block, const RunTable& rt, int& region) {
+  __shared__ int s_pos[CHUNK];
+  __shared__ int s_adr[CHUNK];
+  region = -1;
+  if (block >= rt.counters[0]) return -1;
+  const int4 raw = *reinterpret_cast<const int4*>(rt.chunks + block);
+  Chunk ch;
+  ch.region = raw.x; ch.wg0 = raw.y; ch.pos0 = raw.z; ch.count = raw.w;
+  region = ch.region;
+  const Run* row = rt.runs + int64_t(ch.region) * rt.num_wg;
+  const int t = threadIdx.x;
+  const int nb = min(CHUNK, rt.num_wg - ch.wg0);
+  if (t < nb) {
+    const int2 e = *reinterpret_cast<const int2*>(row + ch.wg0 + t);
+    s_pos[t] = e.x;
+    s_adr[t] = e.y;
+  }
+  __syncthreads();
+  if (t >= ch.count) return -1;
+  const int pos = ch.pos0 + t;
+  int lo = 0, hi = nb;
+  while (hi - lo > 1) {
+    const int mid = (lo + hi) >> 1;
+    if (s_pos[mid] <= pos) lo = mid; else hi = mid;
+  }
+  int p0 = s_pos[lo], adr = s_adr[lo];
+  if (lo == nb - 1 && ch.wg0 + nb < rt.num_wg) {
+    int glo = ch.wg0 + lo, ghi = rt.num_wg;
+    while (ghi - glo > 1) {
+      const int mid = (glo + ghi) >> 1;
+      if (row[mid].pos <= pos) glo = mid; else ghi = mid;
+    }
+    p0 = row[glo].pos;
+    adr = row[glo].addr;
+  }
+  return adr + (pos - p0);
+}
+
+__global__ __launch_bounds__(CHUNK) void count_binned_kernel(MapArgs a, RegionGrid rg, RunTable rt, int* tile_hist,
+                                                           QueryCache* qcache) {
   extern __shared__ int s_win[];
   const int WIN_TILES = rg.win * rg.win;
-  int region, first, count;
-  if (!locate_chunk(blockIdx.x, rg, region_start, chunk_start, region, first, count)) return;
+  int region;
+  const int rec = locate_record(blockIdx.x, rt, region);
+  if (region < 0) return;
   for (int e = threadIdx.x; e < WIN_TILES; e += CHUNK) s_win[e] = 0;
   __syncthreads();
   const Window w(rg, region);
@@ -386,9 +429,13 @@
   };
   int i = 0;
   bool wide = false;
-  if (int(threadIdx.x) < count) {
-    i = order[first + threadIdx.x];
-    const GridQuery q = grid_query(a.points + 7 * int64_t(i), a.Wp, a.Hp, a.tile_size, a.thr);
+  if (rec >= 0) {
+    const uint4* src = reinterpret_cast<const uint4*>(rt.binned + rec);
+    const uint4 b0 = src[0], b1 = src[1];
+    const float g[7] = {__uint_as_float(b0.x), __uint_as_float(b0.y), __uint_as_float(b0.z), __uint_as_float(b0.w),
+                        __uint_as_float(b1.x), __uint_as_float(b1.y), __uint_as_float(b1.z)};
+    i = int(b1.w);
+    const GridQuery q = grid_query(g, a.Wp, a.Hp, a.tile_size, a.thr);
     wide = q.span_x * q.span_y > WIDE_SPAN;
     QueryCache qc;
     qc.accept = 0ull;
@@ -403,7 +450,7 @@
             add_tile(tx + q.min_tx, ty + q.min_ty);
           }
     }
-    *reinterpret_cast<uint4*>(qcache + first + threadIdx.x) = *reinterpret_cast<const uint4*>(&qc);
+    *reinterpret_cast<uint4*>(qcache + int64_t(blockIdx.x) * CHUNK + threadIdx.x) = *reinterpret_cast<const uint4*>(&qc);
   }
   for_each_wide_tile(a, i, __ballot(wide), [&](int) { return add_tile; });
   __syncthreads();
@@ -417,30 +464,34 @@
   }
 }
 
-__global__ __launch_bounds__(CHUNK) void emit_binned_kernel(MapArgs a, RegionGrid rg, const int* order,
-                                                          const int* region_start, const int* chunk_start,
-                                                          int* cursors, uint64_t* pairs, const QueryCache* qcache) {
+__global__ __launch_bounds__(CHUNK) void emit_binned_kernel(MapArgs a, RegionGrid rg, RunTable rt, int* cursors,
+                                                          uint64_t* pairs, const QueryCache* qcache) {
   extern __shared__ int s_dyn[];
   const int WIN_TILES = rg.win * rg.win;
   int* s_cnt = s_dyn;
   int* s_base = s_dyn + WIN_TILES;
-  int region, first, count;
-  if (!locate_chunk(blockIdx.x, rg, region_start, chunk_start, region, first, count)) return;
+  int region;
+  const int rec = locate_record(blockIdx.x, rt, region);
+  if (region < 0) return;
   for (int e = threadIdx.x; e < WIN_TILES; e += CHUNK) s_cnt[e] = 0;
   __syncthreads();
   const Window w(rg, region);
-  const bool active = int(threadIdx.x) < count;
+  const bool active = rec >= 0;
   unsigned long long accept = 0ull;
   int min_tx = 0, min_ty = 0, span_x = 1;
   bool wide = false;
   int i = 0;
+  uint64_t pair = 0;
   auto count_tile = [&](int gx, int gy) {
     int e;
     if (w.slot(gx, gy, e)) atomicAdd(&s_cnt[e], 1);
   };
   if (active) {
-    i = order[first + threadIdx.x];
-    const uint4 raw = *reinterpret_cast<const uint4*>(qcache + first + threadIdx.x);
+    const uint2 key = *reinterpret_cast<const uint2*>(rt.keys + rec);
+    i = int(key.x);
+    const float depth = a.depth ? a.depth[i] : __uint_as_float(key.y);
+    pair = (uint64_t(depth_key(depth, a.depth16 != 0)) << 32) | uint64_t(key.x);
+    const uint4 raw = *reinterpret_cast<const uint4*>(qcache + int64_t(blockIdx.x) * CHUNK + threadIdx.x);
     const QueryCache qc = *reinterpret_cast<const QueryCache*>(&raw);
     wide = (qc.y & QC_WIDE) != 0u;
     if (!wide) {
@@ -475,48 +526,60 @@
     }
     pairs[slot] = pair;
   };
-  auto pair_of = [&](int gi) {
-    return (uint64_t(depth_key(a.depth[gi], a.depth16 != 0)) << 32) | uint64_t(uint32_t(gi));
-  };
-  if (active && !wide) {
-    const uint64_t pair = pair_of(i);
+  if (active && !wide)
     for_each_accepted(accept, span_x, [&](int tx, int ty) { place(tx + min_tx, ty + min_ty, pair); });
-  }
-  for_each_wide_tile(a, i, wide_lanes, [&](int gi) {
-    const uint64_t pair = pair_of(gi);
-    return [&place, pair](int gx, int gy) { place(gx, gy, pair); };
+  for_each_wide_tile(a, i, wide_lanes, [&](int src) {
+    const uint64_t wide_pair = (uint64_t(uint32_t(__shfl(int(pair >> 32), src))) << 32) |
+                               uint64_t(uint32_t(__shfl(int(pair & 0xffffffffull), src)));
+    return [&place, wide_pair](int gx, int gy) { place(gx, gy, wide_pair); };
   });
 }
 
 struct MapScratch {
-  int* hist; int* cursors; int* region_of; int* order; int* region_count; int* region_start; int* part;
-  int* chunk_start;
+  int* hist; int* cursors;
+  int* entered;
+  int* counters;
+  Run* runs;
+  Chunk* chunks;
   QueryCache* qcache;
+  BinRecord* binned;
+  BinKey* keys;
   int* touched_blocks;
   int* block_start;
   char* end;
 };
-int64_t part_entries(int64_t v, int64_t num_tiles) {
-  const int64_t regions = num_tiles < MAX_REGIONS ? (num_tiles < 1 ? 1 : num_tiles) : MAX_REGIONS;
-  return regions * gs_div_up(v > 0 ? v : 1, BIN);
-}
+int64_t max_regions(int64_t num_tiles) { return num_tiles < MAX_REGIONS ? (num_tiles < 1 ? 1 : num_tiles) : MAX_REGIONS; }
+int64_t run_entries(int64_t v, int64_t num_tiles) { return max_regions(num_tiles) * gs_div_up(v > 0 ? v : 1, BIN); }
+int64_t max_chunks(int64_t v, int64_t num_tiles) { return gs_div_up(v, CHUNK) + max_regions(num_tiles); }
 MapScratch carve(void* scratch, int64_t v, int64_t num_tiles) {
   char* p = static_cast<char*>(scratch);
   MapScratch m;
   auto take = [&](int64_t bytes) { int* r = reinterpret_cast<int*>(p); p += gs_align_up(bytes, 256); return r; };
   m.hist = take(num_tiles * 4);
   m.cursors = take(num_tiles * 4);
-  m.region_of = take(v * 4);
-  m.order = take(v * 4);
-  m.region_count = take((MAX_REGIONS + 1) * 4);
-  m.region_start = take((MAX_REGIONS + 1) * 4);
-  m.chunk_start = take((MAX_REGIONS + 1) * 4);
-  m.part = take(part_entries(v, num_tiles) * 4);
-  m.qcache = reinterpret_cast<QueryCache*>(take(v * int64_t(sizeof(QueryCache))));
+  m.entered = take(v * 4);
+  m.counters = take(NUM_COUNTERS * 4);
+  m.runs = reinterpret_cast<Run*>(take(run_entries(v, num_tiles) * int64_t(sizeof(Run))));
+  m.chunks = reinterpret_cast<Chunk*>(take(max_chunks(v, num_tiles) * int64_t(sizeof(Chunk))));
+  m.qcache = reinterpret_cast<QueryCache*>(take(max_chunks(v, num_tiles) * CHUNK * int64_t(sizeof(QueryCache))));
+  m.binned = reinterpret_cast<BinRecord*>(take(v * int64_t(sizeof(BinRecord))));
+  m.keys = reinterpret_cast<BinKey*>(take(v * int64_t(sizeof(BinKey))));
   m.touched_blocks = take((gs_div_up(v > 0 ? v : 1, BIN) + 1) * 4);
   m.block_start = take((gs_div_up(v > 0 ? v : 1, BIN) + 1) * 4);
   m.end = p;
   return m;
+}
+BinOut bin_out(const MapScratch& m, bool want_entered) {
+  BinOut o;
+  o.binned = m.binned; o.keys = m.keys; o.runs = m.runs; o.entered = want_entered ? m.entered : nullptr;
+  o.touched_blocks = m.touched_blocks; o.block_start = m.block_start;
+  return o;
+}
+RunTable run_table(const MapScratch& m, int64_t v) {
+  RunTable rt;
+  rt.binned = m.binned; rt.keys = m.keys; rt.runs = m.runs; rt.chunks = m.chunks; rt.counters = m.counters;
+  rt.num_wg = int(gs_div_up(v > 0 ? v : 1, BIN));
+  return rt;
 }
 RegionGrid make_grid(const MapArgs& a) {
   RegionGrid rg;
@@ -531,12 +594,10 @@
   return rg;
 }
 
-bool bin_with_atomics(int64_t num_wg, const RegionGrid& rg) { return num_wg * rg.num_regions <= (int64_t(1) << 16); }
-
-__global__ __launch_bounds__(1024) void touched_write_kernel(const int* block_start, const int* region_of,
+__global__ __launch_bounds__(1024) void touched_write_kernel(const int* block_start, const int* entered,
                                                              const int* block_counts, int* touched, int* count_out) {
   const int i = block_start[blockIdx.x] + int(threadIdx.x);
-  const bool flag = i < block_start[blockIdx.x + 1] && region_of[i] >= 0;
+  const bool flag = i < block_start[blockIdx.x + 1] && entered[i] >= 0;
   const GsCompactSlot k = gs_stable_compact<16>(flag, nullptr, block_counts, int(blockIdx.x));
   if (flag) touched[k.slot] = i;
   if (count_out && blockIdx.x == gridDim.x - 1 && threadIdx.x == 0) *count_out = k.first + k.total;
@@ -583,7 +644,7 @@
 
 extern "C" int64_t gs_map_touched_offset(int64_t v, int64_t num_tiles) {
   const MapScratch m = carve(nullptr, v, num_tiles);
-  return reinterpret_cast<char*>(m.order) - static_cast<char*>(nullptr);
+  return reinterpret_cast<char*>(m.entered) - static_cast<char*>(nullptr);
 }
 
 extern "C" int gs_map_touched_list(int64_t v, const int32_t* v_dev, int64_t num_tiles, const void* scratch,
@@ -607,7 +668,7 @@
   GS_REQUIRE(touched_out, GS_ERR_INVALID_ARGUMENT, "gs_map_touched_list: touched_out is NULL");
   const MapScratch m = carve(const_cast<void*>(scratch), v, num_tiles);
   const int* block_counts = m.touched_blocks;
-  hipLaunchKernelGGL(touched_write_kernel, dim3(nb), dim3(1024), 0, s, m.block_start, m.region_of, block_counts,
+  hipLaunchKernelGGL(touched_write_kernel, dim3(nb), dim3(1024), 0, s, m.block_start, m.entered, block_counts,
                      touched_out, count_out);
   if (owner_counts) {
     GS_REQUIRE(!owned_rows || (owner >= 0 && owner < world), GS_ERR_INVALID_ARGUMENT,
@@ -624,9 +685,8 @@
   if (int rc = fill_args(a, n, nullptr, nullptr, plan->width, plan->height, plan->cfg, 0, plan->shard)) return rc;
   GS_REQUIRE(a.sh.local_rows > 0 && plan->scratch, GS_ERR_INVALID_ARGUMENT, "gs_map_bin_counters: nothing to bin");
   const MapScratch m = carve(plan->scratch, n, int64_t(a.tiles_wide) * a.sh.local_rows);
-  const bool atomics = bin_with_atomics(gs_div_up(n > 0 ? n : 1, BIN), make_grid(a));
-  *words = atomics ? m.region_count : nullptr;
-  *count = atomics ? MAX_REGIONS + 1 : 0;
+  *words = m.counters;
+  *count = NUM_COUNTERS;
   return GS_OK;
 }
 
@@ -643,8 +703,7 @@
   const MapScratch m = carve(plan->scratch, c->n, num_tiles);
   const unsigned vb = unsigned(gs_div_up(c->n, BIN));
   hipLaunchKernelGGL(compact_bin_kernel, dim3(vb), dim3(BIN), 0, static_cast<hipStream_t>(stream), *c, a, rg, int(vb),
-                     m.region_of, m.part, m.touched_blocks, m.block_start,
-                     bin_with_atomics(vb, rg) ? m.region_count : nullptr);
+                     bin_out(m, plan->shard != nullptr));
   GS_CHECK_LAUNCH("gs_map_compact_bin");
   return GS_OK;
 }
@@ -684,32 +743,20 @@
   if (v > 0) {
     GS_REQUIRE(points, GS_ERR_INVALID_ARGUMENT, "gs_map_prepare: points is NULL");
     const unsigned vb = unsigned(gs_div_up(v, BIN));
-    const bool atomics = bin_with_atomics(vb, rg);
     if (!binned) {
-      if (atomics)
-        if (int rc = gs_memset_async(m.region_count, size_t(MAX_REGIONS + 1) * 4, s,
-                                     "gs_map_prepare: hipMemsetAsync failed"))
-          return rc;
-      hipLaunchKernelGGL(region_count_kernel, dim3(vb), dim3(BIN), 0, s, a, rg, int(vb), m.region_of, m.part,
-                         m.touched_blocks, m.block_start, atomics ? m.region_count : nullptr);
-    }
-    if (!atomics) {
-      hipLaunchKernelGGL(region_part_scan_kernel, dim3(rg.num_regions), dim3(1024), 0, s, int(vb), m.part,
-                         m.region_count);
-      hipLaunchKernelGGL(region_scan_kernel, dim3(1), dim3(1024), 0, s, rg.num_regions, m.region_count,
-                         m.region_start, m.chunk_start);
-    }
-    hipLaunchKernelGGL(region_scatter_kernel, dim3(vb), dim3(BIN), 0, s, rg, int(vb), m.region_of, m.part,
-                       m.region_count, m.region_start, m.chunk_start, m.block_start, m.order, hist, num_tiles,
-                       atomics ? 0 : 1);
+      if (int rc = gs_memset_async(m.counters, size_t(NUM_COUNTERS) * 4, s, "gs_map_prepare: hipMemsetAsync failed"))
+        return rc;
+      hipLaunchKernelGGL(region_bin_kernel, dim3(vb), dim3(BIN), 0, s, a, rg, int(vb), bin_out(m, true));
+    }
+    hipLaunchKernelGGL(region_runs_kernel, dim3(rg.num_regions), dim3(1024), 0, s, int(vb), m.runs, m.counters,
+                       m.chunks, hist, num_tiles);
     hipLaunchKernelGGL(count_binned_kernel, dim3(unsigned(gs_div_up(v, CHUNK)) + unsigned(rg.num_regions)), dim3(CHUNK),
-                       size_t(rg.win) * rg.win * 4, s, a, rg, m.order,
-                       m.region_start, m.chunk_start, hist, m.qcache);
+                       size_t(rg.win) * rg.win * 4, s, a, rg, run_table(m, v), hist, m.qcache);
     GS_CHECK_LAUNCH("gs_map_prepare/count");
   }
   hipLaunchKernelGGL(map_scan_kernel, dim3(tile_order ? 2 : 1), dim3(1024), 0, s, num_tiles, hist,
                      reinterpret_cast<int2*>(tile_ranges), cursors, counts_out, k_capacity, tile_order, v_dev,
-                     counts_host, v > 0 ? m.region_start + rg.num_regions : nullptr);
+                     counts_host, v > 0 ? m.counters + 1 : nullptr);
   GS_CHECK_LAUNCH("gs_map_prepare/scan");
   return GS_OK;
 }
@@ -719,6 +766,14 @@
                              int32_t use_depth16, const int32_t* tile_ranges, int32_t* overlap_to_point,
                              uint64_t* sorted_keys, void* pair_scratch, const GsRowShard* shard, void* scratch,
                              int64_t scratch_bytes, void* stream) {
+  return gs_map_finish_ex(v, v_dev, k, max_tile_count, points, depth, width, height, cfg, use_depth16, tile_ranges,
+                          overlap_to_point, sorted_keys, pair_scratch, shard, scratch, scratch_bytes, 0, stream);
+}
+
+int gs_map_finish_ex(int64_t v, const int32_t* v_dev, int64_t k, int32_t max_tile_count, const float* points,
+                     const float* depth, int32_t width, int32_t height, const GsRasterConfig* cfg, int32_t use_depth16,
+                     const int32_t* tile_ranges, int32_t* overlap_to_point, uint64_t* sorted_keys, void* pair_scratch,
+                     const GsRowShard* shard, void* scratch, int64_t scratch_bytes, int binned, void* stream) {
   MapArgs a;
   if (int rc = fill_args(a, v, points, depth, width, height, cfg, use_depth16, shard)) return rc;
   a.v_dev = v_dev;
@@ -733,9 +788,9 @@
   int* cursors = m.cursors;
   const RegionGrid rg = make_grid(a);
   uint64_t* pairs = static_cast<uint64_t*>(pair_scratch);
+  if (binned) a.depth = nullptr;
   hipLaunchKernelGGL(emit_binned_kernel, dim3(unsigned(gs_div_up(v, CHUNK)) + unsigned(rg.num_regions)), dim3(CHUNK),
-                     size_t(rg.win) * rg.win * 8, s,
-                     a, rg, m.order, m.region_start, m.chunk_start, cursors, pairs, m.qcache);
+                     size_t(rg.win) * rg.win * 8, s, a, rg, run_table(m, v), cursors, pairs, m.qcache);
   GS_CHECK_LAUNCH("gs_map_finish/emit");
   return gs_map_sort_tiles(num_tiles, tile_ranges, pairs, overlap_to_point, sorted_keys, use_depth16, max_tile_count, s);
 }
```

New measurement: 3996 (median of 2 runs). No clear change (-0.1%).
